# jannerm/ddpo

Measured on AMD Instinct MI355X. Metric: sampled images/sec (512^2, 50 DDIM steps), higher is better.
Workload: dtype f32 (f16mx: f16 MFMA + MX-fp8 cross terms on the long-reduction conv/GEMM layers, bf16x3-split MFMA elsewhere); 1 GPU; BASELINE configs[1]: compressed-animals geometry, sd15 U-Net+VAE (random init), 512x512, 50 DDIM steps, CFG 5.0, eta 1.0, sample_batch_size 8/GPU, VAE decode included; parallelism=dp1, global_batch=8

## Files before the change

### ddpo_amd/csrc/gemm_bf16.hip

```cpp
#include "common.h"
#include <cstdlib>
#include <type_traits>

#ifdef DDPO_KLOOP_TIMING
__device__ unsigned long long ddpo_dbg_t[2 * 16384 * 8];
#define DBG_T(i)                                                                                      \
  do {                                                                                                \
    if (threadIdx.x == 0) {                                                                           \
      const int w_ = (blockIdx.x + gridDim.x * blockIdx.y) & 16383;                                   \
      ddpo_dbg_t[w_ * 8 + (i)] = __builtin_amdgcn_s_memtime();                                        \
      ddpo_dbg_t[w_ * 8 + 4 + (i)] = __builtin_amdgcn_s_memrealtime();                                \
    }                                                                                                 \
  } while (0)
#define DBG_ABL(bit) ((d.splits >> 4) & (bit))
#define DBG_WDECL unsigned long long dbg_w0_ = 0, dbg_wacc_ = 0, dbg_bacc_ = 0
#define DBG_W0() do { dbg_w0_ = __builtin_amdgcn_s_memtime(); } while (0)
#define DBG_WMID() do { const unsigned long long n_ = __builtin_amdgcn_s_memtime(); dbg_wacc_ += n_ - dbg_w0_; dbg_w0_ = n_; } while (0)
#define DBG_W1() do { dbg_bacc_ += __builtin_amdgcn_s_memtime() - dbg_w0_; } while (0)
#define DBG_WSTORE()                                                                 \
  do {                                                                               \
    if (threadIdx.x == 0) {                                                          \
      const int w_ = (blockIdx.x + gridDim.x * blockIdx.y) & 16383;                  \
      ddpo_dbg_t[(16384 + w_) * 8 + 0] = dbg_wacc_;                                  \
      ddpo_dbg_t[(16384 + w_) * 8 + 1] = dbg_bacc_;                                  \
    }                                                                                \
  } while (0)
extern "C" int ddpo_debug_kloop_times(unsigned long long* host, int n_wg) {
  (void)n_wg;
  return hipMemcpyFromSymbol(host, HIP_SYMBOL(ddpo_dbg_t), (size_t)2 * 16384 * 8 * sizeof(unsigned long long)) == hipSuccess ? 0 : -1;
}
#else
#define DBG_T(i) do { } while (0)
#define DBG_ABL(bit) 0
#define DBG_WDECL do { } while (0)
#define DBG_W0() do { } while (0)
#define DBG_WMID() do { } while (0)
#define DBG_W1() do { } while (0)
#define DBG_WSTORE() do { } while (0)
#endif

typedef __bf16 bf16x8 __attribute__((ext_vector_type(8)));
typedef float f32x16 __attribute__((ext_vector_type(16)));
typedef _Float16 f16x8 __attribute__((ext_vector_type(8)));
typedef int i32x8 __attribute__((ext_vector_type(8)));
typedef int i32x4 __attribute__((ext_vector_type(4)));

#define BF_BK 32
#define BF_THREADS 256

__device__ __forceinline__ void split2(float a, float b, uint32_t& hi, uint32_t& lo) {
  hi = cvt_pk_bf16(a, b);
  lo = cvt_pk_bf16(a - __uint_as_float(hi << 16), b - __uint_as_float(hi & 0xFFFF0000u));
}

__device__ __forceinline__ f32x16 mx_mfma(const i32x8 a, const i32x8 b, const f32x16 c, int sa, int opb, int sb) {
  switch (opb) {
    case 0: return __builtin_amdgcn_mfma_scale_f32_32x32x64_f8f6f4(a, b, c, 1, 0, 0, sa, 0, sb);
    case 1: return __builtin_amdgcn_mfma_scale_f32_32x32x64_f8f6f4(a, b, c, 1, 0, 0, sa, 1, sb);
    case 2: return __builtin_amdgcn_mfma_scale_f32_32x32x64_f8f6f4(a, b, c, 1, 0, 0, sa, 2, sb);
    default: return __builtin_amdgcn_mfma_scale_f32_32x32x64_f8f6f4(a, b, c, 1, 0, 0, sa, 3, sb);
  }
}

__device__ __forceinline__ int swz_off(int row, int chunk) { return row * 64 + ((chunk ^ ((row >> 2) & 3)) << 4); }

__device__ __forceinline__ void st_out4(float* p, const float4 v) {
  *reinterpret_cast<float4*>(p) = v;
}

__device__ __forceinline__ void store_planes4(const ddpo_gemm_desc& d, int64_t row, int col, const float4 v) {
  if (d.planes_fmt == 1) {
    mx_store4(d.out_hi, d.out_lo, row, col, d.ld_planes, d.M, v);
    return;
  }
  uint2 h, l;
  split4(v, h, l);
  const int64_t o = plane_off(row, col, d.ld_planes, d.M);
  *reinterpret_cast<uint2*>(d.out_hi + o) = h;
  *reinterpret_cast<uint2*>(d.out_lo + o) = l;
}

constexpr int epi_gcd(int a, int b) { return b == 0 ? a : epi_gcd(b, a % b); }
template <int NIT, int LPR, int WTN, int NBMAX = 10>
struct EpiRows {
  static constexpr int PER = LPR / epi_gcd(64, LPR);
  static constexpr int NB = (NIT % 10 == 0 && NBMAX >= 10) ? 10 : (NIT >= 16 && NIT % 8 == 0 && NBMAX >= 8 ? 8 : (NIT % 5 == 0 && NBMAX >= 5 ? 5 : (NIT % 4 == 0 ? 4 : 1)));
  static constexpr int LB = NIT % 5 == 0 ? 5 : (NIT % 4 == 0 ? 4 : 1);
  float4 bv[PER];
  float4 ex[NB];
  bool any;
  __device__ __forceinline__ void init(const ddpo_gemm_desc& d, int col_base, int lane) {
    any = d.bias || d.rowbias || d.residual || d.alpha != 1.0f;
    if (!any) return;
#pragma unroll
    for (int j = 0; j < PER; ++j) {
      const int e = j * 64 + lane, rr = e / LPR;
      const int colc = min(col_base + (e - rr * LPR) * 4, d.N - 4);
      bv[j] = d.bias ? *reinterpret_cast<const float4*>(d.bias + colc) : make_float4(0.f, 0.f, 0.f, 0.f);
    }
  }
  __device__ __forceinline__ void fetch(const ddpo_gemm_desc& d, int b0, int row_base, int col_base, int lane) {
    if (!d.residual && !d.rowbias) return;
    asm volatile("" : "+v"(lane));
#pragma unroll
    for (int i = 0; i < NB; ++i) {
      const int e = (b0 + i) * 64 + lane, rr = e / LPR;
      const int rowc = min(row_base + rr, d.M - 1), colc = min(col_base + (e - rr * LPR) * 4, d.N - 4);
      ex[i] = d.residual ? *reinterpret_cast<const float4*>(d.residual + (int64_t)rowc * d.ld_res + colc)
                         : *reinterpret_cast<const float4*>(d.rowbias + (int64_t)(rowc / d.rows_per_batch) * d.ld_rowbias + colc);
    }
  }
  __device__ __forceinline__ void combine(const ddpo_gemm_desc& d, float* cw, int b0, int row_base, int col_base, int lane) {
    const bool both = d.residual && d.rowbias;
    asm volatile("" : "+v"(lane));
#pragma unroll
    for (int i = 0; i < NB; ++i) {
      const int it = b0 + i;
      const int e = it * 64 + lane, rr = e / LPR, lcol = (e - rr * LPR) * 4;
      float4 v = *reinterpret_cast<const float4*>(cw + rr * WTN + lcol);
      const float4 b4 = bv[it % PER];
      v.x = d.alpha * v.x + b4.x; v.y = d.alpha * v.y + b4.y; v.z = d.alpha * v.z + b4.z; v.w = d.alpha * v.w + b4.w;
      if (both) {
        const int rowc = min(row_base + rr, d.M - 1), colc = min(col_base + lcol, d.N - 4);
        const float4 rb = *reinterpret_cast<const float4*>(d.rowbias + (int64_t)(rowc / d.rows_per_batch) * d.ld_rowbias + colc);
        v.x += rb.x; v.y += rb.y; v.z += rb.z; v.w += rb.w;
      }
      if (d.residual || d.rowbias) { v.x += ex[i].x; v.y += ex[i].y; v.z += ex[i].z; v.w += ex[i].w; }
      *reinterpret_cast<float4*>(cw + rr * WTN + lcol) = v;
    }
  }
  __device__ __forceinline__ void combine_all(const ddpo_gemm_desc& d, float* cw, int row_base, int col_base, int lane) {
    if (!any) return;
#pragma unroll
    for (int b0 = 0; b0 < NIT; b0 += NB) {
      if (b0) fetch(d, b0, row_base, col_base, lane);
      combine(d, cw, b0, row_base, col_base, lane);
    }
  }
  __device__ __forceinline__ static void emit(const ddpo_gemm_desc& d, const float* cw, int row_base, int col_base, int lane) {
#pragma unroll
    for (int b0 = 0; b0 < NIT; b0 += LB) {
      asm volatile("" : "+v"(lane));
      float4 v[LB];
#pragma unroll
      for (int i = 0; i < LB; ++i) {
        const int e = (b0 + i) * 64 + lane, rr = e / LPR;
        v[i] = *reinterpret_cast<const float4*>(cw + rr * WTN + (e - rr * LPR) * 4);
      }
#pragma unroll
      for (int i = 0; i < LB; ++i) {
        const int e = (b0 + i) * 64 + lane, rr = e / LPR;
        const int row = row_base + rr, col = col_base + (e - rr * LPR) * 4;
        if (row >= d.M || col >= d.N) continue;
        if (d.out) st_out4(d.out + (int64_t)row * d.ld_out + col, v[i]);
        if (d.out_hi) store_planes4(d, row, col, v[i]);
      }
    }
  }
  __device__ __forceinline__ static void partials(const ddpo_gemm_desc& d, const float* cw, float* pp, int row_base, int col_base, int lane) {
#pragma unroll
    for (int it = 0; it < NIT; ++it) {
      const int e = it * 64 + lane, rr = e / LPR, lcol = (e - rr * LPR) * 4;
      const int row = row_base + rr, col = col_base + lcol;
      if (row >= d.M || col >= d.N) continue;
      *reinterpret_cast<float4*>(pp + (int64_t)row * d.N + col) = *reinterpret_cast<const float4*>(cw + rr * WTN + lcol);
    }
  }
};

template <int BM, int BN, int NPASS, bool AFFINE>
__global__ void __launch_bounds__(BF_THREADS) gemm_conv_bf16_kernel(const ddpo_gemm_desc d, const uint16_t* __restrict__ w_hi,
                                                                   const uint16_t* __restrict__ w_lo, int ldw, int tiles_m,
                                                                   int tiles_n, int nblk, int kt_per_split,
                                                                   float* __restrict__ part) {
  constexpr int BK = BF_BK;
  constexpr int TM = BM / 64, TN = BN / 64;
  constexpr int AROWS = BM / 32;
  constexpr int BCH = BN / 64;
  constexpr int NPL = (NPASS == 3) ? 2 : 1;
  constexpr int A_BYTES = BM * 64, B_BYTES = BN * 64;
  extern __shared__ __attribute__((aligned(16))) char smem[];
  constexpr int STAGE = NPL * (A_BYTES + B_BYTES);
  const int t = threadIdx.x, lane = t & 63, wid = t >> 6;
  const int wm = wid >> 1, wn = wid & 1;

  int bid = blockIdx.x;
  {
    const int xcd = bid & 7, idx = bid >> 3;
    const int q = nblk >> 3, r = nblk & 7;
    bid = (xcd < r ? xcd * (q + 1) : r * (q + 1) + (xcd - r) * q) + idx;
  }
  constexpr int GROUP_M = 8;
  const int per_group = GROUP_M * tiles_n;
  const int group = bid / per_group, in_group = bid - group * per_group;
  const int gm0 = group * GROUP_M;
  const int gsz = min(tiles_m - gm0, GROUP_M);
  const int tile_n = in_group / gsz, tile_m = gm0 + (in_group - tile_n * gsz);
  const int m0 = tile_m * BM, n0 = tile_n * BN;

  const bool conv = d.ksize > 0;
  const int VH = d.upsample ? d.H * 2 : d.H, VW = d.upsample ? d.W * 2 : d.W;
  const bool zins = d.upsample == 2;

  const int kq = t & 7;
  const float* arow_ptr[AROWS];
  uint32_t amask[AROWS];
  int aiy0[AROWS], aix0[AROWS];
  int64_t abase[AROWS];
#pragma unroll
  for (int i = 0; i < AROWS; ++i) {
    const int m = m0 + (t >> 3) + 32 * i;
    const bool valid = m < d.M;
    amask[i] = 0;
    if (conv) {
      const int ohw = d.OH * d.OW;
      const int mm = valid ? m : 0;
      const int b = mm / ohw, rem = mm - b * ohw;
      const int oy = rem / d.OW, ox = rem - oy * d.OW;
      const int iy0 = oy * d.stride - d.pad, ix0 = ox * d.stride - d.pad;
      abase[i] = (int64_t)b * d.H * d.W;
      aiy0[i] = iy0; aix0[i] = ix0;
      arow_ptr[i] = d.src + (abase[i] + (int64_t)iy0 * d.W + ix0) * d.ld_src;
      if (AFFINE && valid) {
        for (int ky = 0; ky < d.ksize; ++ky)
          for (int kx = 0; kx < d.ksize; ++kx)
            if (iy0 + ky >= 0 && iy0 + ky < d.H && ix0 + kx >= 0 && ix0 + kx < d.W) amask[i] |= 1u << (ky * d.ksize + kx);
      }
    } else {
      abase[i] = 0; aiy0[i] = aix0[i] = 0;
      arow_ptr[i] = d.src + (int64_t)m * d.ld_src;
      amask[i] = valid ? 1u : 0u;
    }
  }
  const int nk_total = (d.K + BK - 1) / BK;
  const int kt0 = blockIdx.y * kt_per_split;
  const int nk = min(kt_per_split, nk_total - kt0);
// ... 121 lines not shown
      for (int i = 0; i < TM; ++i) {
        ah[i] = *reinterpret_cast<const bf16x8*>(sa + a_ld[ks][i]);
        if (NPASS == 3) al[i] = *reinterpret_cast<const bf16x8*>(sa + A_BYTES + a_ld[ks][i]);
      }
#pragma unroll
      for (int j = 0; j < TN; ++j) {
        bh[j] = *reinterpret_cast<const bf16x8*>(sb + b_ld[ks][j]);
        if (NPASS == 3) bl[j] = *reinterpret_cast<const bf16x8*>(sb + B_BYTES + b_ld[ks][j]);
      }
#pragma unroll
      for (int i = 0; i < TM; ++i)
#pragma unroll
        for (int j = 0; j < TN; ++j) {
          if (NPASS == 3) {
            acc[i][j] = __builtin_amdgcn_mfma_f32_32x32x16_bf16(al[i], bh[j], acc[i][j], 0, 0, 0);
            acc[i][j] = __builtin_amdgcn_mfma_f32_32x32x16_bf16(ah[i], bl[j], acc[i][j], 0, 0, 0);
          }
          acc[i][j] = __builtin_amdgcn_mfma_f32_32x32x16_bf16(ah[i], bh[j], acc[i][j], 0, 0, 0);
        }
    }
  };

  load_tile(0, s0);
  store_tile(0, s0);
  load_tile(1, s0);
  __syncthreads();
  const int nk2 = (nk + 1) & ~1;
#pragma unroll 1
  for (int kt = 0; kt < nk2; kt += 2) {
    load_tile(kt + 2, s1);
    compute(0);
    store_tile(1, s0);
    __syncthreads();
    load_tile(kt + 3, s0);
    compute(1);
    store_tile(0, s1);
    __syncthreads();
  }

  if (part) {
    float* pp = part + (int64_t)blockIdx.y * d.M * d.N;
#pragma unroll
    for (int i = 0; i < TM; ++i)
#pragma unroll
      for (int j = 0; j < TN; ++j) {
        const int col = n0 + wn * (BN / 2) + j * 32 + (lane & 31);
        if (col >= d.N) continue;
#pragma unroll
        for (int r = 0; r < 16; ++r) {
          const int row = m0 + wm * (BM / 2) + i * 32 + (r & 3) + 8 * (r >> 2) + 4 * khalf;
          if (row < d.M) pp[(int64_t)row * d.N + col] = acc[i][j][r];
        }
      }
    return;
  }
#pragma unroll
  for (int i = 0; i < TM; ++i) {
#pragma unroll
    for (int j = 0; j < TN; ++j) {
      const int col = n0 + wn * (BN / 2) + j * 32 + (lane & 31);
      if (col >= d.N) continue;
      const float bv = d.bias ? d.bias[col] : 0.f;
#pragma unroll
      for (int r = 0; r < 16; ++r) {
        const int row = m0 + wm * (BM / 2) + i * 32 + (r & 3) + 8 * (r >> 2) + 4 * khalf;
        if (row >= d.M) continue;
        float v = d.alpha * acc[i][j][r] + bv;
        if (d.rowbias) v += d.rowbias[(int64_t)(row / d.rows_per_batch) * d.ld_rowbias + col];
        if (d.residual) v += d.residual[(int64_t)row * d.ld_res + col];
        d.out[(int64_t)row * d.ld_out + col] = v;
      }
    }
  }
}

typedef unsigned int u32x4 __attribute__((ext_vector_type(4)));
typedef unsigned int u32x2 __attribute__((ext_vector_type(2)));
#define BUF_OOB 0x80000000u

__device__ __forceinline__ __amdgpu_buffer_rsrc_t make_rsrc(const void* p) {
  return __builtin_amdgcn_make_buffer_rsrc(const_cast<void*>(p), 0, 0x7FFFFFFF, 0x00020000);
}

template <int BM, int BN, int NPASS, int ABL = 0, int WM = 2, int WN = 2, bool DEEP = true, int APL = 0>
__global__ void __launch_bounds__(64 * WM * WN, (BM * BN <= 128 * 64 ? 3 : 1)) gemm_conv_bf16_buf_kernel(const ddpo_gemm_desc d, const uint16_t* __restrict__ w_hi,
                                                                       const uint16_t* __restrict__ w_lo, int ldw, int tiles_m,
                                                                       int tiles_n, int nblk, int kt_per_split,
                                                                       float* __restrict__ part) {
  constexpr int BK = BF_BK;
  constexpr int THREADS = 64 * WM * WN;
  constexpr int WTM = BM / WM, WTN = BN / WN;
  constexpr int TM = WTM / 32, TN = WTN / 32;
  constexpr int AR = THREADS / 8, BR = THREADS / 4;
  constexpr int AROWS = BM / AR;
  constexpr int BCH = (BN + BR - 1) / BR;
  constexpr bool BFULL = (BN % BR) == 0;
  static_assert(BM % AR == 0 && WTM % 32 == 0 && WTN % 32 == 0, "tile / wave-grid mismatch");
  constexpr bool MX = NPASS == 4;
  static_assert(!MX || APL == 3 || APL == 7, "the f16mx datapath exists on the plane-fed 128-row tiles (APL 3) and on the tall tile (APL 7)");
  constexpr int NPL = (NPASS == 3 || NPASS == 4) ? 2 : 1;
  constexpr int A_BYTES = BM * 64, B_BYTES = BN * 64;
  extern __shared__ __attribute__((aligned(16))) char smem[];
  constexpr int STAGE = NPL * (A_BYTES + B_BYTES);
  const int t = threadIdx.x, lane = t & 63, wid = t >> 6;
  const int wm = wid / WN, wn = wid % WN;
  DBG_T(0);
  DBG_WDECL;

  int bid = blockIdx.x;
  {
    const int xcd = bid & 7, idx = bid >> 3;
    const int q = nblk >> 3, r = nblk & 7;
    bid = (xcd < r ? xcd * (q + 1) : r * (q + 1) + (xcd - r) * q) + idx;
  }
  constexpr int GROUP_M = 8;
  const int per_group = GROUP_M * tiles_n;
  const int group = bid / per_group, in_group = bid - group * per_group;
  const int gm0 = group * GROUP_M;
  const int gsz = min(tiles_m - gm0, GROUP_M);
  const int tile_n = in_group / gsz, tile_m = gm0 + (in_group - tile_n * gsz);
  const int m0 = tile_m * BM, n0 = tile_n * BN;

  const bool conv = d.ksize > 0;
  const int VH = d.upsample ? d.H * 2 : d.H, VW = d.upsample ? d.W * 2 : d.W;
  const bool zins = d.upsample == 2;
  const int cin = conv ? d.Cin : d.K;
  const int ntaps = conv ? d.ksize * d.ksize : 1;

  f32x16 acc[TM][TN];
#pragma unroll
  for (int i = 0; i < TM; ++i)
#pragma unroll
    for (int j = 0; j < TN; ++j)
#pragma unroll
      for (int r = 0; r < 16; ++r) acc[i][j][r] = 0.f;

  const int khalf = lane >> 5;
  static_assert((WTM % 32) == 0 && (WTN % 32) == 0, "wave sub-tiles are whole 32-row blocks");
  const int a_ld0 = swz_off(wm * WTM + (lane & 31), khalf), b_ld0 = swz_off(wn * WTN + (lane & 31), khalf);
  const int a_ld1 = a_ld0 ^ 32, b_ld1 = b_ld0 ^ 32;

  struct Frag { bf16x8 ah[TM], al[TM], bh[TN], bl[TN]; i32x8 a8[TM], b8[TN]; };
  auto ldfrag_at = [&](const char* sa, const char* sb, int ks, Frag& f) {
    const char* pa = sa + (ks ? a_ld1 : a_ld0);
    const char* pb = sb + (ks ? b_ld1 : b_ld0);
#pragma unroll
    for (int i = 0; i < TM; ++i) {
      f.ah[i] = *reinterpret_cast<const bf16x8*>(pa + i * 2048);
      if (NPASS == 3) f.al[i] = *reinterpret_cast<const bf16x8*>(pa + A_BYTES + i * 2048);
      if (MX && ks) {
        const i32x4 x = *reinterpret_cast<const i32x4*>(sa + a_ld0 + A_BYTES + i * 2048), y = *reinterpret_cast<const i32x4*>(sa + a_ld1 + A_BYTES + i * 2048);
        f.a8[i] = i32x8{x[0], x[1], x[2], x[3], y[0], y[1], y[2], y[3]};
      }
    }
#pragma unroll
    for (int j = 0; j < TN; ++j) {
      f.bh[j] = *reinterpret_cast<const bf16x8*>(pb + j * 2048);
      if (NPASS == 3) f.bl[j] = *reinterpret_cast<const bf16x8*>(pb + B_BYTES + j * 2048);
      if (MX && ks) {
        const i32x4 x = *reinterpret_cast<const i32x4*>(sb + b_ld0 + B_BYTES + j * 2048), y = *reinterpret_cast<const i32x4*>(sb + b_ld1 + B_BYTES + j * 2048);
        f.b8[j] = i32x8{x[0], x[1], x[2], x[3], y[0], y[1], y[2], y[3]};
      }
    }
  };
  auto ldfrag = [&](int cur, int ks, Frag& f) {
    const char* sa = smem + cur * STAGE;
    ldfrag_at(sa, sa + NPL * A_BYTES, ks, f);
  };
  int mx_sa = 0, mx_sbp[(TN + 3) / 4];
  if constexpr (MX) {
    mx_sa = khalf ? 127 - 11 : 127;
#pragma unroll
    for (int q = 0; q < (TN + 3) / 4; ++q) mx_sbp[q] = 0;
#pragma unroll
    for (int j = 0; j < TN; ++j) {
      const int n = n0 + wn * WTN + j * 32 + (lane & 31);
      const int sc = n < d.N ? (int)d.w_scale[n] : 127;
      mx_sbp[j >> 2] |= (khalf ? sc : sc - 11) << (8 * (j & 3));
    }
  }
  auto mma = [&](const Frag& f, int tbeg, int tend, int ks = 0) {
#pragma unroll
    for (int i = 0; i < TM; ++i) {
#pragma unroll
      for (int j = 0; j < TN; ++j) {
        if (i * TN + j < tbeg || i * TN + j >= tend) continue;
        if constexpr (MX) {
          acc[i][j] = __builtin_amdgcn_mfma_f32_32x32x16_f16(__builtin_bit_cast(f16x8, f.ah[i]), __builtin_bit_cast(f16x8, f.bh[j]), acc[i][j], 0, 0, 0);
          if (ks) acc[i][j] = mx_mfma(f.a8[i], f.b8[j], acc[i][j], mx_sa, j & 3, mx_sbp[j >> 2]);
          continue;
        }
        if (NPASS == 3) {
          acc[i][j] = __builtin_amdgcn_mfma_f32_32x32x16_bf16(f.al[i], f.bh[j], acc[i][j], 0, 0, 0);
          acc[i][j] = __builtin_amdgcn_mfma_f32_32x32x16_bf16(f.ah[i], f.bl[j], acc[i][j], 0, 0, 0);
        }
        if constexpr (NPASS == 5) acc[i][j] = __builtin_amdgcn_mfma_f32_32x32x16_f16(__builtin_bit_cast(f16x8, f.ah[i]), __builtin_bit_cast(f16x8, f.bh[j]), acc[i][j], 0, 0, 0);
        else acc[i][j] = __builtin_amdgcn_mfma_f32_32x32x16_bf16(f.ah[i], f.bh[j], acc[i][j], 0, 0, 0);
      }
    }
  };

  if constexpr (APL != 0) {
    static_assert(NPASS == 1 || NPASS == 3 || NPASS == 4 || NPASS == 5, "the plane-fed path: bf16x3 / f16mx (two planes per operand) or single-pass bf16 / f16 (one)");
    constexpr int NW = WM * WN, PAIRS = NPL == 2 ? NW / 2 : NW;
    constexpr int GA = BM / 16, GB = BN / 16;
    static_assert(NW % 2 == 0 && GA % PAIRS == 0 && (NPL == 1 || GB % PAIRS == 0), "pieces must divide evenly over the loader groups");
    constexpr int NA = GA / PAIRS, NB = (GB + PAIRS - 1) / PAIRS;
    constexpr int B_LDS = NB * PAIRS * 1024;
    const int wv = __builtin_amdgcn_readfirstlane(wid);
    const int plane = NPL == 2 ? (wv & 1) : 0, pr = NPL == 2 ? (wv >> 1) : wv;
    const int lr = lane >> 2;
    const uint32_t lc16 = (uint32_t)((lane & 3) ^ ((lane >> 4) & 3)) * 16u;
    const uint64_t a_ptr = reinterpret_cast<uint64_t>(plane ? reinterpret_cast<const void*>(d.w) : reinterpret_cast<const void*>(d.src));
    const uint64_t w_ptr = reinterpret_cast<uint64_t>(plane ? w_lo : w_hi);
    const u32x4 rs_a = {(uint32_t)a_ptr, (uint32_t)(a_ptr >> 32) & 0xFFFFu, 0x7FFFFFFFu, 0x00020000u};
    const u32x4 rs_w = {(uint32_t)w_ptr, (uint32_t)(w_ptr >> 32) & 0xFFFFu, 0x7FFFFFFFu, 0x00020000u};
    const uint32_t lds0 = (uint32_t)(uintptr_t)((__attribute__((address_space(3))) char*)smem);
    const uint32_t lds_a = lds0 + plane * A_BYTES + pr * 1024;
    const uint32_t lds_w = lds0 + NPL * A_BYTES + plane * B_BYTES + pr * 1024;

    const uint32_t a_row_b = d.ld_src == 0 ? 64u : (uint32_t)d.ld_src * 2u;
    const uint32_t a_kt_b = d.ld_src == 0 ? (uint32_t)(conv ? d.B * d.H * d.W : d.M) * 64u : (uint32_t)(BK * 2);
    int aiy0[NA], aix0[NA], apix[NA];
    uint32_t avoff[NA], bvoff[NB];
#pragma unroll
    for (int i = 0; i < NA; ++i) {
      const int m = m0 + 16 * (pr + PAIRS * i) + lr;
      const bool valid = m < d.M;
      if (conv) {
        const int ohw = d.OH * d.OW;
        const int mm = valid ? m : 0;
        const int b = mm / ohw, rem = mm - b * ohw;
        const int oy = rem / d.OW, ox = rem - oy * d.OW;
        aiy0[i] = valid ? oy * d.stride - d.pad : -(1 << 24);
        aix0[i] = ox * d.stride - d.pad;
        apix[i] = b * d.H * d.W;
        avoff[i] = BUF_OOB;
      } else {
        aiy0[i] = aix0[i] = apix[i] = 0;
        avoff[i] = valid ? (uint32_t)m * a_row_b + lc16 : BUF_OOB;
      }
    }
    auto set_tap = [&](int tap) {
      const int ky = d.ksize == 3 ? (tap * 11) >> 5 : 0;
      const int kx = d.ksize == 3 ? tap - ky * 3 : 0;
#pragma unroll
      for (int i = 0; i < NA; ++i) {
        const int iy = aiy0[i] + ky, ix = aix0[i] + kx;
        const bool ok = (unsigned)iy < (unsigned)VH && (unsigned)ix < (unsigned)VW && !(zins && ((iy | ix) & 1));
        const int sy = d.upsample ? (iy >> 1) : iy, sx = d.upsample ? (ix >> 1) : ix;
        const uint32_t off = (uint32_t)(apix[i] + sy * d.W + sx) * a_row_b + lc16;
        avoff[i] = ok ? off : BUF_OOB;
      }
    };
    const uint32_t w_row_b = d.w_layout == 1 ? 64u : (uint32_t)ldw * 2u;
    const uint32_t w_kt_b = d.w_layout == 1 ? (uint32_t)d.N * 64u : (uint32_t)(BK * 2);
#pragma unroll
    for (int i = 0; i < NB; ++i) {
      const int n = n0 + 16 * (pr + PAIRS * i) + lr;
      bool in_tile = true;
      if constexpr (GB % PAIRS != 0) in_tile = pr + PAIRS * i < GB;
      bvoff[i] = (n < d.N && in_tile) ? (uint32_t)n * w_row_b + lc16 : BUF_OOB;
    }
    const int nk_total = d.K / BK;
    const int kt0 = blockIdx.y * kt_per_split;
    const int nk = min(kt_per_split, nk_total - kt0);
    int tap = (kt0 * BK) / cin, cib = kt0 * BK - tap * cin;
    if (conv) set_tap(tap);
    int kt_next = kt0;

    auto fill = [&](int stage) {
      const uint32_t so_a = (uint32_t)(cib >> 5) * a_kt_b, so_w = (uint32_t)kt_next * w_kt_b;
      const uint32_t la = lds_a + stage * STAGE, lw = lds_w + stage * STAGE;
      if (!DBG_ABL(4) || (kt_next - kt0) % 9 < 2) {
#pragma unroll
      for (int i = 0; i < NA; ++i)
        asm volatile("s_nop 4\n\ts_mov_b32 m0, %0\n\ts_nop 0\n\tbuffer_load_dwordx4 %1, %2, %3 offen lds"
                     :: "s"(la + i * (PAIRS * 1024)), "v"(avoff[i]), "s"(rs_a), "s"(so_a) : "memory");
      }
#pragma unroll
      for (int i = 0; i < NB; ++i)
        asm volatile("s_nop 4\n\ts_mov_b32 m0, %0\n\ts_nop 0\n\tbuffer_load_dwordx4 %1, %2, %3 offen lds"
                     :: "s"(lw + i * (PAIRS * 1024)), "v"(bvoff[i]), "s"(rs_w), "s"(so_w) : "memory");
      ++kt_next;
      cib += BK;
      if (cib >= cin) {
        cib = 0; ++tap;
        if (conv && tap < ntaps) set_tap(tap);
      }
    };
    if constexpr (APL == 5 || APL == 6) {
      const bool late = (d.splits & 1) != 0 && wv >= NW / 2;
      auto step4 = [&](int kt, auto cur_c) {
        constexpr int cur = decltype(cur_c)::value;
        DBG_W0();
        asm volatile("s_waitcnt vmcnt(0) lgkmcnt(0)" ::: "memory");
        DBG_WMID();
        __builtin_amdgcn_s_barrier();
        DBG_W1();
        if (kt == 0) DBG_T(1);
        if (kt + 1 < nk && !late && !DBG_ABL(1)) fill(cur ^ 1);
        Frag g;
        ldfrag(cur, 0, g);
        if (!DBG_ABL(2)) mma(g, 0, TM * TN);
        if (kt + 1 < nk && late && !DBG_ABL(1)) fill(cur ^ 1);
        ldfrag(cur, 1, g);
        if (!DBG_ABL(2)) mma(g, 0, TM * TN);
        if (DBG_ABL(2)) asm volatile("" :: "v"(g.ah[0]), "v"(g.bl[TN - 1]), "v"(g.al[TM - 1]), "v"(g.bh[0]));
      };
      {
        const bool rot = wv >= NW / 2;
        fill(0);
        Frag g;
        if (!rot) {
          int kt = 0;
#pragma unroll 1
          for (; kt + 1 < nk; kt += 2) {
            step4(kt, std::integral_constant<int, 0>{});
            step4(kt + 1, std::integral_constant<int, 1>{});
          }
          if (kt < nk) step4(kt, std::integral_constant<int, 0>{});
        } else {
          auto step5 = [&](int kt, auto cur_c) {
            constexpr int cur = decltype(cur_c)::value;
            asm volatile("s_waitcnt vmcnt(0) lgkmcnt(0)" ::: "memory");
            __builtin_amdgcn_s_barrier();
            __builtin_amdgcn_sched_barrier(0);
            if (kt > 0) mma(g, 0, TM * TN);
            __builtin_amdgcn_sched_barrier(0);
            if (kt + 1 < nk) fill(cur ^ 1);
            ldfrag(cur, 0, g);
            mma(g, 0, TM * TN);
            ldfrag(cur, 1, g);
// ... 302 lines not shown
      char* st = smem + buf * STAGE;
#pragma unroll
      for (int i = 0; i < AROWS; ++i) {
        uint2 hi, lo;
        split4(sg.a[i], hi, lo);
        *reinterpret_cast<uint2*>(st + a_st[i]) = hi;
        if (NPASS == 3) *reinterpret_cast<uint2*>(st + A_BYTES + a_st[i]) = lo;
      }
      char* sb = st + NPL * A_BYTES;
#pragma unroll
      for (int i = 0; i < BCH; ++i) {
        if (!BFULL && (t >> 2) + BR * i >= BN) continue;
        *reinterpret_cast<uint4*>(sb + b_st[i]) = sg.bh[i];
        if (NPASS == 3) *reinterpret_cast<uint4*>(sb + B_BYTES + b_st[i]) = sg.bl[i];
      }
    };

    Frag f0, f1;
    constexpr int TT = TM * TN, TH = TT / 2;

    if (ABL & 32) {
#pragma unroll
      for (int i = 0; i < AROWS; ++i) s0.a[i] = make_float4(1.f, 1.f, 1.f, 1.f);
#pragma unroll
      for (int i = 0; i < BCH; ++i) s0.bh[i] = s0.bl[i] = make_uint4(0x3f803f80u, 0x3f803f80u, 0x3f803f80u, 0x3f803f80u);
      store_tile(0, s0);
    } else {
      load_tile(0, s0);
      store_tile(0, s0);
      if (DEEP) load_tile(1, s0);
    }
    __syncthreads();
    DBG_T(1);
    ldfrag(0, 0, f0);
    if (ABL & 8) ldfrag(0, 1, f1);
    if (ABL & 1) s1 = s0;
    const int nk2 = nk & ~1;
#pragma unroll 1
    for (int kt = 0; kt < nk2; kt += 2) {
      if (!(ABL & 1)) { if (DEEP) load_tile(kt + 2, s1); else load_tile(kt + 1, s0); }
      if (!(ABL & 8)) ldfrag(0, 1, f1);
      mma(f0, 0, TT);
      if (!(ABL & 2)) store_tile(1, s0);
      __builtin_amdgcn_sched_barrier(0);
      mma(f1, 0, TH);
      __builtin_amdgcn_sched_barrier(0);
      if (!(ABL & 4)) __syncthreads();
      if (!(ABL & 8)) ldfrag(1, 0, f0);
      __builtin_amdgcn_sched_barrier(0);
      mma(f1, TH, TT);
      if (!(ABL & 1)) { if (DEEP) load_tile(kt + 3, s0); else load_tile(kt + 2, s0); }
      if (!(ABL & 8)) ldfrag(1, 1, f1);
      mma(f0, 0, TT);
      if (!(ABL & 2)) { if (DEEP) store_tile(0, s1); else store_tile(0, s0); }
      __builtin_amdgcn_sched_barrier(0);
      mma(f1, 0, TH);
      __builtin_amdgcn_sched_barrier(0);
      if (!(ABL & 4)) __syncthreads();
      if (!(ABL & 8)) ldfrag(0, 0, f0);
      __builtin_amdgcn_sched_barrier(0);
      mma(f1, TH, TT);
    }
    if (nk & 1) {
      ldfrag(0, 1, f1);
      mma(f0, 0, TT);
      mma(f1, 0, TT);
    }

  }

  DBG_T(2);
  DBG_WSTORE();
  const bool vec_ok = ((d.N | d.ld_out) & 3) == 0 && (reinterpret_cast<uintptr_t>(d.out) & 15) == 0 &&
                      (!d.residual || ((d.ld_res & 3) == 0 && (reinterpret_cast<uintptr_t>(d.residual) & 15) == 0)) &&
                      (!d.rowbias || ((d.ld_rowbias & 3) == 0 && (reinterpret_cast<uintptr_t>(d.rowbias) & 15) == 0)) &&
                      (!d.bias || (reinterpret_cast<uintptr_t>(d.bias) & 15) == 0);
  if constexpr (BM == 256) {
    if (vec_ok) {
      constexpr int LPR = WTN / 4;
      constexpr int NIT = 32 * LPR / 64;
      static_assert((32 * LPR) % 64 == 0, "32-row pass must be a whole number of wave instructions");
      __syncthreads();
      float* cw = reinterpret_cast<float*>(smem) + wid * (32 * WTN);
      float* pp = part ? part + (int64_t)blockIdx.y * d.M * d.N : nullptr;
      using Epi = EpiRows<NIT, LPR, WTN, 5>;
      Epi ep;
      const int colb = n0 + wn * WTN;
      static_assert(TM == 2, "the tall tile's output stage is written for two 32-row passes per wave");
      if constexpr (APL == 6) {
        static_assert(WN == 2 && WTN == 160, "value / gate wave pairs of 160 columns");
        const int oc0 = (n0 / 320) * 160;
        float bj[TN];
#pragma unroll
        for (int j = 0; j < TN; ++j) bj[j] = d.bias ? d.bias[colb + j * 32 + (lane & 31)] : 0.f;
        const float* ca = reinterpret_cast<const float*>(smem) + (wid & ~1) * (32 * WTN);
        const float* cg = ca + 32 * WTN;
        auto gpass = [&](auto IH) {
          constexpr int ih = decltype(IH)::value;
          if (ih > 0) __syncthreads();
#pragma unroll
          for (int j = 0; j < TN; ++j)
#pragma unroll
            for (int r = 0; r < 16; ++r) {
              cw[((r & 3) + 8 * (r >> 2) + 4 * khalf) * WTN + j * 32 + (lane & 31)] = acc[ih][j][r] + bj[j];
            }
          __syncthreads();
          constexpr int GL = WTN / 4;
          int ln = lane;
          asm volatile("" : "+v"(ln));
#pragma unroll
          for (int it = 0; it < 16 * GL / 64; ++it) {
            const int e = it * 64 + ln, rr = wn * 16 + e / GL, c4 = (e - (e / GL) * GL) * 4;
            const float4 a = *reinterpret_cast<const float4*>(ca + rr * WTN + c4);
            const float4 g = *reinterpret_cast<const float4*>(cg + rr * WTN + c4);
            const float4 o = make_float4(a.x * gelu_tanh_f(g.x), a.y * gelu_tanh_f(g.y), a.z * gelu_tanh_f(g.z), a.w * gelu_tanh_f(g.w));
            const int row = m0 + wm * WTM + ih * 32 + rr, col = oc0 + c4;
            if (row >= d.M) continue;
            if (d.aux_out) {
              float* pa = d.aux_out + (int64_t)row * d.N + col;
              *reinterpret_cast<float4*>(pa) = a;
              *reinterpret_cast<float4*>(pa + (d.N >> 1)) = g;
            }
            if (d.out) st_out4(d.out + (int64_t)row * d.ld_out + col, o);
            if (d.out_hi) store_planes4(d, row, col, o);
          }
        };
        gpass(std::integral_constant<int, 0>{});
        gpass(std::integral_constant<int, 1>{});
        DBG_T(3);
        return;
      }
      auto pass = [&](auto IH) {
        constexpr int ih = decltype(IH)::value;
        const int rowb = m0 + wm * WTM + ih * 32;
        if (ih > 0 && !pp) ep.fetch(d, 0, rowb, colb, lane);
#pragma unroll
        for (int j = 0; j < TN; ++j)
#pragma unroll
          for (int r = 0; r < 16; ++r)
            cw[((r & 3) + 8 * (r >> 2) + 4 * khalf) * WTN + j * 32 + (lane & 31)] = acc[ih][j][r];
        if (pp) {
          Epi::partials(d, cw, pp, rowb, colb, lane);
        } else {
          if (ih == 0) { ep.init(d, colb, lane); ep.fetch(d, 0, rowb, colb, lane); }
          ep.combine_all(d, cw, rowb, colb, lane);
          Epi::emit(d, cw, rowb, colb, lane);
        }
      };
      pass(std::integral_constant<int, 0>{});
      pass(std::integral_constant<int, 1>{});
      DBG_T(3);
      return;
    }
  }
  if (vec_ok && !(ABL & 16) && BM != 256) {
    constexpr int LPR = WTN / 4;
    constexpr int NIT = WTM * LPR / 64;
    static_assert((WTM * LPR) % 64 == 0, "wave sub-tile must be a whole number of 1 KiB rows");
    __syncthreads();
    float* cw = reinterpret_cast<float*>(smem) + wid * (WTM * WTN);
    using Epi = EpiRows<NIT, LPR, WTN>;
    Epi ep;
    const int rowb = m0 + wm * WTM, colb = n0 + wn * WTN;
    const bool plain = !part && !(BN == 128 && WN == 2 && WM == 2 && d.epilogue == 1);
    if (plain) { ep.init(d, colb, lane); ep.fetch(d, 0, rowb, colb, lane); }
#pragma unroll
    for (int i = 0; i < TM; ++i)
#pragma unroll
      for (int j = 0; j < TN; ++j)
#pragma unroll
        for (int r = 0; r < 16; ++r)
          cw[(i * 32 + (r & 3) + 8 * (r >> 2) + 4 * khalf) * WTN + j * 32 + (lane & 31)] = acc[i][j][r];
    if (BN == 128 && WN == 2 && WM == 2 && d.epilogue == 1) {
      const int q = (n0 + wn * 64) >> 6;
      const int gc = (lane & 7) * 4, grow = lane >> 3;
      const float4 ba = d.bias ? *reinterpret_cast<const float4*>(d.bias + q * 64 + gc) : make_float4(0.f, 0.f, 0.f, 0.f);
      const float4 bg = d.bias ? *reinterpret_cast<const float4*>(d.bias + q * 64 + 32 + gc) : make_float4(0.f, 0.f, 0.f, 0.f);
#pragma unroll
      for (int it = 0; it < 8; ++it) {
        const int rr = it * 8 + grow;
        const int row = m0 + wm * 64 + rr;
        if (row >= d.M) continue;
        const float4 a = *reinterpret_cast<const float4*>(cw + rr * 64 + gc);
        const float4 g = *reinterpret_cast<const float4*>(cw + rr * 64 + 32 + gc);
        float4 o;
        o.x = (a.x + ba.x) * gelu_tanh_f(g.x + bg.x); o.y = (a.y + ba.y) * gelu_tanh_f(g.y + bg.y);
        o.z = (a.z + ba.z) * gelu_tanh_f(g.z + bg.z); o.w = (a.w + ba.w) * gelu_tanh_f(g.w + bg.w);
        if (d.aux_out) {
          float* pa = d.aux_out + (int64_t)row * d.N + q * 32 + gc;
          *reinterpret_cast<float4*>(pa) = make_float4(a.x + ba.x, a.y + ba.y, a.z + ba.z, a.w + ba.w);
          *reinterpret_cast<float4*>(pa + (d.N >> 1)) = make_float4(g.x + bg.x, g.y + bg.y, g.z + bg.z, g.w + bg.w);
        }
        if (d.out) st_out4(d.out + (int64_t)row * d.ld_out + q * 32 + gc, o);
        if (d.out_hi) store_planes4(d, row, q * 32 + gc, o);
      }
      DBG_T(3);
      return;
    }
    if (part) {
      Epi::partials(d, cw, part + (int64_t)blockIdx.y * d.M * d.N, rowb, colb, lane);
    } else {
      ep.combine_all(d, cw, rowb, colb, lane);
      Epi::emit(d, cw, rowb, colb, lane);
    }
    DBG_T(3);
    return;
  }
  if (part) {
    float* pp = part + (int64_t)blockIdx.y * d.M * d.N;
#pragma unroll
    for (int i = 0; i < TM; ++i)
#pragma unroll
      for (int j = 0; j < TN; ++j) {
        const int col = n0 + wn * WTN + j * 32 + (lane & 31);
        if (col >= d.N) continue;
#pragma unroll
        for (int r = 0; r < 16; ++r) {
          const int row = m0 + wm * WTM + i * 32 + (r & 3) + 8 * (r >> 2) + 4 * khalf;
          if (row < d.M) pp[(int64_t)row * d.N + col] = acc[i][j][r];
        }
      }
    DBG_T(3);
    return;
  }
#pragma unroll
  for (int i = 0; i < TM; ++i) {
#pragma unroll
    for (int j = 0; j < TN; ++j) {
      const int col = n0 + wn * WTN + j * 32 + (lane & 31);
      if (col >= d.N) continue;
      const float bv = d.bias ? d.bias[col] : 0.f;
#pragma unroll
      for (int r = 0; r < 16; ++r) {
        const int row = m0 + wm * WTM + i * 32 + (r & 3) + 8 * (r >> 2) + 4 * khalf;
        if (row >= d.M) continue;
        if ((ABL & 16) && (r | i | j)) { if (acc[i][j][r] == 123.456f) d.out[0] = 1.f; continue; }
        float v = d.alpha * acc[i][j][r] + bv;
        if (d.rowbias) v += d.rowbias[(int64_t)(row / d.rows_per_batch) * d.ld_rowbias + col];
        if (d.residual) v += d.residual[(int64_t)row * d.ld_res + col];
        d.out[(int64_t)row * d.ld_out + col] = v;
      }
    }
  }
  DBG_T(3);
}

__global__ void __launch_bounds__(256) splitk_reduce_kernel(const ddpo_gemm_desc d, const float* __restrict__ part, int splits) {
  const int n4 = d.N >> 2;
  const int64_t total = (int64_t)d.M * n4, mn = (int64_t)d.M * d.N;
  for (int64_t i = (int64_t)blockIdx.x * blockDim.x + threadIdx.x; i < total; i += (int64_t)gridDim.x * blockDim.x) {
    const int row = (int)(i / n4), col = (int)(i - (int64_t)row * n4) << 2;
    float4 a = *reinterpret_cast<const float4*>(part + (int64_t)row * d.N + col);
    for (int s = 1; s < splits; ++s) {
      const float4 b = *reinterpret_cast<const float4*>(part + s * mn + (int64_t)row * d.N + col);
      a.x += b.x; a.y += b.y; a.z += b.z; a.w += b.w;
    }
    float v[4] = {a.x, a.y, a.z, a.w};
#pragma unroll
    for (int e = 0; e < 4; ++e) {
      float x = d.alpha * v[e] + (d.bias ? d.bias[col + e] : 0.f);
      if (d.rowbias) x += d.rowbias[(int64_t)(row / d.rows_per_batch) * d.ld_rowbias + col + e];
      if (d.residual) x += d.residual[(int64_t)row * d.ld_res + col + e];
      v[e] = x;
      if (d.out) d.out[(int64_t)row * d.ld_out + col + e] = x;
    }
    if (d.out_hi) store_planes4(d, row, col, make_float4(v[0], v[1], v[2], v[3]));
  }
}

static bool planes_out_ok(const ddpo_gemm_desc& d) {
  if (!d.out_hi) return d.out != nullptr && !d.out_lo;
  if (!d.out_lo || d.ld_planes < 0 || (d.ld_planes & 3)) return false;
  if ((reinterpret_cast<uintptr_t>(d.out_hi) | reinterpret_cast<uintptr_t>(d.out_lo)) & 7) return false;
  const int ncols = d.epilogue != 0 ? d.N / 2 : d.N;
  if (d.ld_planes == 0 ? (ncols & 31) != 0 : d.ld_planes < ncols) return false;
  if (d.planes_fmt != 0 && (d.planes_fmt != 1 || (ncols & 31) || (d.ld_planes & 31))) return false;
  if (d.N & 3) return false;
  if (d.out && ((d.ld_out & 3) || (reinterpret_cast<uintptr_t>(d.out) & 15))) return false;
  if (d.residual && ((d.ld_res & 3) || (reinterpret_cast<uintptr_t>(d.residual) & 15))) return false;
  if (d.rowbias && ((d.ld_rowbias & 3) || (reinterpret_cast<uintptr_t>(d.rowbias) & 15))) return false;
  if (d.bias && (reinterpret_cast<uintptr_t>(d.bias) & 15)) return false;
  return true;
}

enum { TC_TALL = 0, TC_WIDE = 1, TC_128 = 2, TC_64 = 3, TC_GENERIC = 4, TC_SPLITK_REDUCE = 5, TC_MX = 6, TC_COUNT = 8 };
static unsigned long long g_tile_launches[TC_COUNT] = {0, 0, 0, 0, 0, 0, 0, 0};
extern "C" int ddpo_gemm_tile_launch_counts(unsigned long long* out_host, int n) {
  if (!out_host || n < TC_COUNT) return DDPO_EINVAL;
  for (int i = 0; i < TC_COUNT; ++i) out_host[i] = __atomic_load_n(&g_tile_launches[i], __ATOMIC_RELAXED);
  return DDPO_OK;
}
static inline void count_tile(int cls) { __atomic_fetch_add(&g_tile_launches[cls], 1ull, __ATOMIC_RELAXED); }

static bool g_force_generic = false;
static bool buf_path_ok(const ddpo_gemm_desc& d, int ldw) {
  if (g_force_generic) return false;
  const int64_t lim = 0x7FFFFFFF;
  if (d.w_layout == 1) ldw = (d.K + 31) / 32 * 32;
  if (d.ksize > 0) {
    if (d.Cin % BF_BK) return false;
    if ((int64_t)d.B * d.H * d.W * (d.ld_src ? d.ld_src : d.Cin) * 4 >= lim) return false;
    const int64_t wbytes = d.w_dgrad ? (int64_t)d.K * d.N * 2 : (int64_t)d.N * ldw * 2;
    if (wbytes >= lim) return false;
  } else {
    if (d.K % BF_BK) return false;
    if ((int64_t)d.M * (d.ld_src ? d.ld_src : d.K) * 4 >= lim || (int64_t)d.N * ldw * 2 >= lim) return false;
  }
  return true;
}
#ifdef DDPO_DEBUG_HOOKS
extern "C" void ddpo_debug_force_generic_gemm(int on) { g_force_generic = on != 0; }
#endif

template <int BM, int BN, int NPASS, int WM = 2, int WN = 2, int APL = 0>
static int launch_bf16(const ddpo_gemm_desc& d, const uint16_t* w_hi, const uint16_t* w_lo, int ldw, float* ws, size_t ws_bytes,
                       hipStream_t st) {
  const int tiles_m = (d.M + BM - 1) / BM, tiles_n = (d.N + BN - 1) / BN;
  const int nblk = tiles_m * tiles_n;
  const int nk_total = (d.K + BF_BK - 1) / BF_BK;
  int splits = 1;
  if (ws && nblk < 192 && nk_total >= 32 && (d.N & 3) == 0 && d.epilogue == 0) {
    splits = (384 + nblk - 1) / nblk;
    if (splits > 8) splits = 8;
    if (splits > nk_total / 8) splits = nk_total / 8;
    while (splits > 1 && (size_t)splits * d.M * d.N * sizeof(float) > ws_bytes) --splits;
  }
  int ktps = (nk_total + splits - 1) / splits;
  ktps = (ktps + 1) & ~1;
  splits = (nk_total + ktps - 1) / ktps;
  float* part = splits > 1 ? ws : nullptr;
  constexpr int NPL = (NPASS == 3 || NPASS == 4) ? 2 : 1;
  size_t lds = (APL == 3) ? NPL * (size_t)(2 * BM + 3 * BN) * 64 : 2 * NPL * (size_t)(BM + BN) * 64;
  if (lds < (size_t)BM * BN * 4) lds = (size_t)BM * BN * 4;
  static bool attr_set = false;
  if (!attr_set) {
    if constexpr (APL == 0) {
      (void)hipFuncSetAttribute(reinterpret_cast<const void*>(&gemm_conv_bf16_kernel<BM, BN, NPASS, true>),
                                hipFuncAttributeMaxDynamicSharedMemorySize, (int)lds);
      (void)hipFuncSetAttribute(reinterpret_cast<const void*>(&gemm_conv_bf16_kernel<BM, BN, NPASS, false>),
                                hipFuncAttributeMaxDynamicSharedMemorySize, (int)lds);
    }
    (void)hipFuncSetAttribute(reinterpret_cast<const void*>(&gemm_conv_bf16_buf_kernel<BM, BN, NPASS, 0, WM, WN, true, APL>),
                              hipFuncAttributeMaxDynamicSharedMemorySize, (int)lds);
    attr_set = true;
  }
  count_tile(BN == 128 ? TC_128 : TC_64);
  if constexpr (NPASS == 4) count_tile(TC_MX);
  if constexpr (APL != 0) {
    hipLaunchKernelGGL((gemm_conv_bf16_buf_kernel<BM, BN, NPASS, 0, WM, WN, true, APL>), dim3(nblk, splits), dim3(64 * WM * WN), lds, st, d, w_hi,
                       w_lo, ldw, tiles_m, tiles_n, nblk, ktps, part);
  } else {
    if (!buf_path_ok(d, ldw)) count_tile(TC_GENERIC);
    if (buf_path_ok(d, ldw))
      hipLaunchKernelGGL((gemm_conv_bf16_buf_kernel<BM, BN, NPASS, 0, WM, WN, true, APL>), dim3(nblk, splits), dim3(64 * WM * WN), lds, st, d, w_hi,
                         w_lo, ldw, tiles_m, tiles_n, nblk, ktps, part);
    else if (d.upsample == 0)
      hipLaunchKernelGGL((gemm_conv_bf16_kernel<BM, BN, NPASS, true>), dim3(nblk, splits), dim3(BF_THREADS), lds, st, d, w_hi, w_lo, ldw,
                         tiles_m, tiles_n, nblk, ktps, part);
    else
      hipLaunchKernelGGL((gemm_conv_bf16_kernel<BM, BN, NPASS, false>), dim3(nblk, splits), dim3(BF_THREADS), lds, st, d, w_hi, w_lo, ldw,
                         tiles_m, tiles_n, nblk, ktps, part);
  }
  DDPO_LAUNCH_CHECK();
  if (splits > 1) {
    int64_t blocks = ((int64_t)d.M * (d.N >> 2) + 255) / 256;
    if (blocks > 4096) blocks = 4096;
    count_tile(TC_SPLITK_REDUCE);
    hipLaunchKernelGGL(splitk_reduce_kernel, dim3((int)blocks), dim3(256), 0, st, d, part, splits);
    DDPO_LAUNCH_CHECK();
  }
  return DDPO_OK;
}


static int wide_splits(const ddpo_gemm_desc& d, bool have_ws, size_t ws_bytes) {
  const int nblk = ((d.M + 127) / 128) * ((d.N + 319) / 320);
  const int nk_total = d.K / BF_BK;
  int splits = 1;
  if (have_ws && nblk <= 192 && nk_total >= 16) {
    splits = (256 + nblk / 2) / nblk;
    if (splits > 8) splits = 8;
    if (splits > nk_total / 8) splits = nk_total / 8;
    if (splits < 1) splits = 1;
    while (splits > 1 && (size_t)splits * d.M * d.N * sizeof(float) > ws_bytes) --splits;
  }
  return splits;
}

template <int NPASS, int APL = 0>
static int launch_bf16_wide(const ddpo_gemm_desc& d, const uint16_t* w_hi, const uint16_t* w_lo, int ldw, float* ws, size_t ws_bytes,
                            hipStream_t st) {
  constexpr int BM = 128, BN = 320, WM = 4, WN = 2;
  const int tiles_m = (d.M + BM - 1) / BM, tiles_n = (d.N + BN - 1) / BN;
  const int nblk = tiles_m * tiles_n;
  const int nk_total = d.K / BF_BK;
  int splits = wide_splits(d, ws != nullptr, ws_bytes);
  int ktps = (nk_total + splits - 1) / splits;
  ktps = (ktps + 1) & ~1;
  splits = (nk_total + ktps - 1) / ktps;
  float* part = splits > 1 ? ws : nullptr;
  const size_t lds = (size_t)BM * BN * 4;
  static bool attr_set = false;
  if (!attr_set) {
    (void)hipFuncSetAttribute(reinterpret_cast<const void*>(&gemm_conv_bf16_buf_kernel<BM, BN, NPASS, 0, WM, WN, true, APL>),
                              hipFuncAttributeMaxDynamicSharedMemorySize, (int)lds);
    attr_set = true;
  }
  count_tile(TC_WIDE);
  if constexpr (NPASS == 4) count_tile(TC_MX);
  hipLaunchKernelGGL((gemm_conv_bf16_buf_kernel<BM, BN, NPASS, 0, WM, WN, true, APL>), dim3(nblk, splits), dim3(64 * WM * WN), lds, st, d, w_hi,
                     w_lo, ldw, tiles_m, tiles_n, nblk, ktps, part);
  DDPO_LAUNCH_CHECK();
  if (splits > 1) {
    int64_t blocks = ((int64_t)d.M * (d.N >> 2) + 255) / 256;
    if (blocks > 4096) blocks = 4096;
    count_tile(TC_SPLITK_REDUCE);
    hipLaunchKernelGGL(splitk_reduce_kernel, dim3((int)blocks), dim3(256), 0, st, d, part, splits);
    DDPO_LAUNCH_CHECK();
  }
  return DDPO_OK;
}

template <int APL, int NPASS = 3>
static int launch_bf16_tall(const ddpo_gemm_desc& d, const uint16_t* w_hi, const uint16_t* w_lo, int ldw, hipStream_t st) {
  constexpr int BM = 256, BN = 320, WM = 4, WN = 2;
  const int tiles_m = (d.M + BM - 1) / BM, tiles_n = (d.N + BN - 1) / BN;
  const int nblk = tiles_m * tiles_n;
  const int nk_total = d.K / BF_BK;
  const size_t lds = 8 * 32 * 160 * 4;
  static bool attr_set = false;
  if (!attr_set) {
    (void)hipFuncSetAttribute(reinterpret_cast<const void*>(&gemm_conv_bf16_buf_kernel<BM, BN, NPASS, 0, WM, WN, true, APL>),
                              hipFuncAttributeMaxDynamicSharedMemorySize, (int)lds);
    attr_set = true;
  }
  count_tile(TC_TALL);
  hipLaunchKernelGGL((gemm_conv_bf16_buf_kernel<BM, BN, NPASS, 0, WM, WN, true, APL>), dim3(nblk, 1), dim3(64 * WM * WN), lds, st, d, w_hi, w_lo, ldw,
                     tiles_m, tiles_n, nblk, nk_total, (float*)nullptr);
  DDPO_LAUNCH_CHECK();
  return DDPO_OK;
}

static int launch_mx_tall(const ddpo_gemm_desc& d, const uint16_t* w16, const uint16_t* w8, hipStream_t st) {
  constexpr int BM = 256, BN = 320, WM = 4, WN = 2;
  const int tiles_m = (d.M + BM - 1) / BM, tiles_n = (d.N + BN - 1) / BN;
  const int nblk = tiles_m * tiles_n;
  const int nk_total = d.K / BF_BK;
  const size_t lds = 8 * 32 * 160 * 4;
  static bool attr_set = false;
  if (!attr_set) {
    (void)hipFuncSetAttribute(reinterpret_cast<const void*>(&gemm_conv_bf16_buf_kernel<BM, BN, 4, 0, WM, WN, true, 7>),
                              hipFuncAttributeMaxDynamicSharedMemorySize, (int)lds);
    attr_set = true;
  }
  count_tile(TC_TALL);
  count_tile(TC_MX);
  hipLaunchKernelGGL((gemm_conv_bf16_buf_kernel<BM, BN, 4, 0, WM, WN, true, 7>), dim3(nblk, 1), dim3(64 * WM * WN), lds, st, d, w16, w8, 0,
                     tiles_m, tiles_n, nblk, nk_total, (float*)nullptr);
  DDPO_LAUNCH_CHECK();
  return DDPO_OK;
}

template <int APL>
static int dispatch_bf16(const ddpo_gemm_desc& d, const uint16_t* w_hi, const uint16_t* w_lo, int ldw, int npass, void* ws, size_t ws_bytes,
                         hipStream_t st) {
  if (d.epilogue != 0) {
    if ((d.epilogue != 1 && d.epilogue != 2) || (d.N & 127) || !buf_path_ok(d, ldw) || d.rowbias || d.residual || d.alpha != 1.0f || d.w_dgrad) return DDPO_EINVAL;
    if ((d.ld_out & 3) || (reinterpret_cast<uintptr_t>(d.out) & 15) || (d.bias && (reinterpret_cast<uintptr_t>(d.bias) & 15))) return DDPO_EINVAL;
    if (reinterpret_cast<uintptr_t>(d.aux_out) & 15) return DDPO_EINVAL;
    if (d.epilogue == 2) {
      if constexpr (APL == 3) {
        if (npass != 3 || d.N % 320 || ((d.N >> 1) & 3)) return DDPO_EINVAL;
        return launch_bf16_tall<6>(d, w_hi, w_lo, ldw, st);
      }
      return DDPO_EINVAL;
    }
    if constexpr (APL == 3) {
      if (npass == 4) return launch_bf16<128, 128, 4, 2, 2, 3>(d, w_hi, w_lo, ldw, nullptr, 0, st);
      if (npass == 1) return launch_bf16<128, 128, 1, 2, 2, 3>(d, w_hi, w_lo, ldw, nullptr, 0, st);
      if (npass == 5) return launch_bf16<128, 128, 5, 2, 2, 3>(d, w_hi, w_lo, ldw, nullptr, 0, st);
    }
    return npass == 3 ? launch_bf16<128, 128, 3, 2, 2, APL>(d, w_hi, w_lo, ldw, nullptr, 0, st) : launch_bf16<128, 128, 1>(d, w_hi, w_lo, ldw, nullptr, 0, st);
  }
  float* wsf = (ws && !(reinterpret_cast<uintptr_t>(ws) & 15)) ? reinterpret_cast<float*>(ws) : nullptr;
  constexpr int wide_mode = 1;
  if constexpr (APL != 0) {
    constexpr int tall_mode = 1;
    const long ntall = (long)((d.M + 255) / 256) * (d.N / 320), nwide = (long)((d.M + 127) / 128) * (d.N / 320);
    const double eff_tall = (double)ntall / (double)(((ntall + 255) / 256) * 256), eff_wide = (double)nwide / (double)(((nwide + 255) / 256) * 256);
    if (tall_mode && npass == 3 && d.N % 320 == 0 && d.epilogue == 0 && ntall >= 200 && eff_tall * 1.08 >= eff_wide)
      return launch_bf16_tall<5>(d, w_hi, w_lo, ldw, st);
    if constexpr (APL == 3) {
      if (npass == 1 && d.N % 320 == 0 && d.epilogue == 0 && ntall >= 200 && eff_tall * 1.08 >= eff_wide)
        return launch_bf16_tall<8, 1>(d, w_hi, w_lo, ldw, st);
      if (npass == 5 && d.N % 320 == 0 && d.epilogue == 0 && ntall >= 200 && eff_tall * 1.08 >= eff_wide)
        return launch_bf16_tall<8, 5>(d, w_hi, w_lo, ldw, st);
      const char* mx_tall_env = getenv("DDPO_MX_TALL");
      if (npass == 4 && !(mx_tall_env && mx_tall_env[0] == '0') && d.N % 320 == 0 && d.epilogue == 0 && ntall >= 200 && eff_tall * 1.08 >= eff_wide)
        return launch_mx_tall(d, w_hi, w_lo, st);
    }
  }
  const int wsplits = wide_splits(d, wsf != nullptr, ws_bytes);
  if (wide_mode && d.N % 320 == 0 && d.M >= 512 && buf_path_ok(d, ldw) && !(d.K / BF_BK < 16 && d.N > 1280) &&
      (long)((d.M + 127) / 128) * (d.N / 320) * wsplits >= 200 &&
      !(wsplits > 1 && d.K / BF_BK < 64)) {
    if constexpr (APL == 3) {
      if (npass == 4) return launch_bf16_wide<4, 3>(d, w_hi, w_lo, ldw, wsf, ws_bytes, st);
      if (npass == 1) return launch_bf16_wide<1, 3>(d, w_hi, w_lo, ldw, wsf, ws_bytes, st);
      if (npass == 5) return launch_bf16_wide<5, 3>(d, w_hi, w_lo, ldw, wsf, ws_bytes, st);
    }
    return npass == 3 ? launch_bf16_wide<3, APL>(d, w_hi, w_lo, ldw, wsf, ws_bytes, st) : launch_bf16_wide<1>(d, w_hi, w_lo, ldw, wsf, ws_bytes, st);
  }
  const long t128 = (long)((d.M + 127) / 128) * ((d.N + 127) / 128);
  constexpr long big_min = 256;
  constexpr int mid64 = 1;
  const bool mid_short = mid64 && t128 < 512 && d.K / BF_BK <= 64;
  const bool big = (d.N % 128 == 0) && t128 >= big_min && !mid_short;
  if constexpr (APL == 3) {
    if (npass == 4)
      return big ? launch_bf16<128, 128, 4, 2, 2, 3>(d, w_hi, w_lo, ldw, wsf, ws_bytes, st) : launch_bf16<128, 64, 4, 2, 2, 3>(d, w_hi, w_lo, ldw, wsf, ws_bytes, st);
    if (npass == 1)
      return big ? launch_bf16<128, 128, 1, 2, 2, 3>(d, w_hi, w_lo, ldw, wsf, ws_bytes, st) : launch_bf16<128, 64, 1, 2, 2, 3>(d, w_hi, w_lo, ldw, wsf, ws_bytes, st);
    if (npass == 5)
      return big ? launch_bf16<128, 128, 5, 2, 2, 3>(d, w_hi, w_lo, ldw, wsf, ws_bytes, st) : launch_bf16<128, 64, 5, 2, 2, 3>(d, w_hi, w_lo, ldw, wsf, ws_bytes, st);
  }
  if (npass == 3)
    return big ? launch_bf16<128, 128, 3, 2, 2, APL>(d, w_hi, w_lo, ldw, wsf, ws_bytes, st) : launch_bf16<128, 64, 3, 2, 2, APL>(d, w_hi, w_lo, ldw, wsf, ws_bytes, st);
  return big ? launch_bf16<128, 128, 1>(d, w_hi, w_lo, ldw, wsf, ws_bytes, st) : launch_bf16<128, 64, 1>(d, w_hi, w_lo, ldw, wsf, ws_bytes, st);
}

extern "C" int ddpo_gemm_conv_fwd_bf16(const ddpo_gemm_desc* dp, const uint16_t* w_hi, const uint16_t* w_lo, int ldw, int npass,
                                       void* ws, size_t ws_bytes, void* stream) {
  if (!dp || !w_hi) return DDPO_EINVAL;
  const ddpo_gemm_desc& d = *dp;
  if (npass != 1 && npass != 3) return DDPO_EINVAL;
  if (npass == 3 && !w_lo) return DDPO_EINVAL;
  if (!d.src || d.M <= 0 || d.N <= 0 || d.K <= 0 || d.ld_src <= 0 || (d.ld_src & 3) || (reinterpret_cast<uintptr_t>(d.src) & 15)) return DDPO_EINVAL;
  if ((reinterpret_cast<uintptr_t>(w_hi) & 15) || (w_lo && (reinterpret_cast<uintptr_t>(w_lo) & 15))) return DDPO_EINVAL;
  if (!planes_out_ok(d) || (d.out_hi && !buf_path_ok(d, ldw))) return DDPO_EINVAL;
  if (d.ksize > 0) {
    if (d.ksize != 1 && d.ksize != 3) return DDPO_EINVAL;
    if ((d.Cin & 7) || d.K != d.ksize * d.ksize * d.Cin || d.M != d.B * d.OH * d.OW) return DDPO_EINVAL;
    if (d.upsample < 0 || d.upsample > 2) return DDPO_EINVAL;
  } else if (d.K & 7) {
    return DDPO_EINVAL;
  }
  if (d.w_layout != 0 && (d.w_layout != 1 || d.w_dgrad)) return DDPO_EINVAL;
  if (d.w_dgrad) {
    if (d.ksize <= 0 || (d.Cin & 7)) return DDPO_EINVAL;
  } else if (d.w_layout == 0 && (ldw < d.K || (ldw & 7))) {
    return DDPO_EINVAL;
  }
  return dispatch_bf16<0>(d, w_hi, w_lo, ldw, npass, ws, ws_bytes, as_stream(stream));
}

extern "C" int ddpo_gemm_conv_fwd_bf16_planes(const ddpo_gemm_desc* dp, const uint16_t* a_hi, const uint16_t* a_lo, int lda,
                                              const uint16_t* w_hi, const uint16_t* w_lo, int ldw, void* ws, size_t ws_bytes,
                                              void* stream) {
  if (!dp || !a_hi || !w_hi || (a_lo == nullptr) != (w_lo == nullptr)) return DDPO_EINVAL;
  const int npass = a_lo ? 3 : 1;
  ddpo_gemm_desc d = *dp;
  if (d.M <= 0 || d.N <= 0 || d.K <= 0 || lda < 0 || (lda & 7) || d.w_dgrad || !planes_out_ok(d)) return DDPO_EINVAL;
  if (npass == 1 && d.epilogue == 2) return DDPO_EINVAL;
  if ((reinterpret_cast<uintptr_t>(a_hi) | reinterpret_cast<uintptr_t>(a_lo) | reinterpret_cast<uintptr_t>(w_hi) |
       reinterpret_cast<uintptr_t>(w_lo)) & 15) return DDPO_EINVAL;
  if (d.w_layout != 0 && d.w_layout != 1) return DDPO_EINVAL;
  if (d.w_layout == 0 && (ldw < d.K || (ldw & 7))) return DDPO_EINVAL;
  if (d.ksize > 0) {
    if (d.ksize != 1 && d.ksize != 3) return DDPO_EINVAL;
    if (d.K != d.ksize * d.ksize * d.Cin || d.M != d.B * d.OH * d.OW || d.upsample < 0 || d.upsample > 2 || (lda && lda < d.Cin)) return DDPO_EINVAL;
  } else if (lda && lda < d.K) {
    return DDPO_EINVAL;
  }
  d.src = reinterpret_cast<const float*>(a_hi);
  d.w = reinterpret_cast<const float*>(a_lo);
  d.ld_src = lda;
  if (!buf_path_ok(d, ldw)) return DDPO_EINVAL;
  d.splits = 1;
#ifdef DDPO_KLOOP_TIMING
  { const char* e = getenv("DDPO_DBG_ABL"); if (e) d.splits |= atoi(e) << 4; }
#endif
  return dispatch_bf16<3>(d, w_hi, w_lo, ldw, npass, ws, ws_bytes, as_stream(stream));
}

extern "C" int ddpo_gemm_conv_fwd_f16mx_planes(const ddpo_gemm_desc* dp, const uint16_t* a16, const uint16_t* a8, int lda,
                                               const uint16_t* w16, const uint16_t* w8, void* ws, size_t ws_bytes, void* stream) {
  if (!dp || !a16 || !w16 || (a8 == nullptr) != (w8 == nullptr) || (a8 && !dp->w_scale)) return DDPO_EINVAL;
  const int npass = a8 ? 4 : 5;
  ddpo_gemm_desc d = *dp;
  if (npass == 5 && d.epilogue == 2) return DDPO_EINVAL;
  if (d.M <= 0 || d.N <= 0 || d.K <= 0 || lda < 0 || (lda & 31) || d.w_dgrad || d.w_layout != 1 || !planes_out_ok(d)) return DDPO_EINVAL;
  if ((reinterpret_cast<uintptr_t>(a16) | reinterpret_cast<uintptr_t>(a8) | reinterpret_cast<uintptr_t>(w16) | reinterpret_cast<uintptr_t>(w8)) & 15)
    return DDPO_EINVAL;
  if (d.ksize > 0) {
    if (d.ksize != 1 && d.ksize != 3) return DDPO_EINVAL;
    if (d.K != d.ksize * d.ksize * d.Cin || d.M != d.B * d.OH * d.OW || d.upsample < 0 || d.upsample > 2 || (lda && lda < d.Cin)) return DDPO_EINVAL;
  } else if (lda && lda < d.K) {
    return DDPO_EINVAL;
  }
  d.src = reinterpret_cast<const float*>(a16);
  d.w = reinterpret_cast<const float*>(a8);
  d.ld_src = lda;
  if (!buf_path_ok(d, 0)) return DDPO_EINVAL;
  d.splits = 1;
#ifdef DDPO_KLOOP_TIMING
  { const char* e = getenv("DDPO_DBG_ABL"); if (e) d.splits |= atoi(e) << 4; }
#endif
  return dispatch_bf16<3>(d, w16, w8, 0, npass, ws, ws_bytes, as_stream(stream));
}

__global__ void __launch_bounds__(256) pack_weights_kernel(const float* __restrict__ w, int K, int N, int Kp,
                                                           uint16_t* __restrict__ fwd_hi, uint16_t* __restrict__ fwd_lo,
                                                           uint16_t* __restrict__ bwd_hi, uint16_t* __restrict__ bwd_lo) {
  __shared__ uint32_t tile[32][33];
  const int k0 = blockIdx.y * 32, n0 = blockIdx.x * 32;
  const int tx = threadIdx.x & 31, ty = threadIdx.x >> 5;
  for (int r = ty; r < 32; r += 8) {
    const int k = k0 + r, n = n0 + tx;
    uint32_t packed = 0;
    if (k < K && n < N) {
      const float x = w[(int64_t)k * N + n];
      const uint32_t h = cvt_pk_bf16(x, 0.f) & 0xFFFFu;
      const float rem = x - __uint_as_float(h << 16);
      const uint32_t l = cvt_pk_bf16(rem, 0.f) & 0xFFFFu;
      packed = h | (l << 16);
      if (bwd_hi) { bwd_hi[(int64_t)k * N + n] = (uint16_t)h; bwd_lo[(int64_t)k * N + n] = (uint16_t)l; }
    }
    tile[r][tx] = packed;
  }
  __syncthreads();
  for (int r = ty; r < 32; r += 8) {
    const int n = n0 + r, k = k0 + tx;
    if (n < N && k < Kp) {
      const uint32_t p = tile[tx][r];
      fwd_hi[(int64_t)n * Kp + k] = (uint16_t)(p & 0xFFFFu);
      fwd_lo[(int64_t)n * Kp + k] = (uint16_t)(p >> 16);
    }
  }
}

__global__ void __launch_bounds__(256) pack_weights_kblocked_kernel(const float* __restrict__ w, int K, int N, uint16_t* __restrict__ fwd_hi,
                                                                    uint16_t* __restrict__ fwd_lo) {
  __shared__ uint32_t tile[32][33];
  const int kb = blockIdx.y, k0 = kb * 32, n0 = blockIdx.x * 32;
  const int tx = threadIdx.x & 31, ty = threadIdx.x >> 5;
  for (int r = ty; r < 32; r += 8) {
    const int k = k0 + r, n = n0 + tx;
    uint32_t packed = 0;
    if (k < K && n < N) {
      const float x = w[(int64_t)k * N + n];
      const uint32_t h = cvt_pk_bf16(x, 0.f) & 0xFFFFu;
      const float rem = x - __uint_as_float(h << 16);
      packed = h | ((cvt_pk_bf16(rem, 0.f) & 0xFFFFu) << 16);
    }
    tile[r][tx] = packed;
  }
  __syncthreads();
  for (int r = ty; r < 32; r += 8) {
    const int n = n0 + r;
    if (n < N) {
      const uint32_t p = tile[tx][r];
      const int64_t o = ((int64_t)kb * N + n) * 32 + tx;
      fwd_hi[o] = (uint16_t)(p & 0xFFFFu);
      fwd_lo[o] = (uint16_t)(p >> 16);
    }
  }
}

extern "C" int ddpo_pack_weights_bf16_kblocked(const float* w, int K, int N, uint16_t* fwd_hi, uint16_t* fwd_lo, void* stream) {
  if (!w || !fwd_hi || !fwd_lo || K <= 0 || N <= 0) return DDPO_EINVAL;
  dim3 grid((N + 31) / 32, (K + 31) / 32);
  hipLaunchKernelGGL(pack_weights_kblocked_kernel, grid, dim3(256), 0, as_stream(stream), w, K, N, fwd_hi, fwd_lo);
  DDPO_LAUNCH_CHECK();
  return DDPO_OK;
}

__global__ void __launch_bounds__(256) pack_weights_kblocked_dgrad_kernel(const float* __restrict__ w, int taps, int Cin, int Cout,
                                                                          uint16_t* __restrict__ hi, uint16_t* __restrict__ lo) {
  const int kb = blockIdx.y, tx = threadIdx.x & 31, ty = threadIdx.x >> 5;
  const int Kd = taps * Cout;
  const int k = kb * 32 + tx;
  const bool kok = k < Kd;
  const int tap = kok ? k / Cout : 0, co = k - tap * Cout;
  const float* src = w + ((int64_t)(taps - 1 - tap) * Cin) * Cout + co;
  for (int r = ty; r < 32; r += 8) {
    const int n = blockIdx.x * 32 + r;
    if (n >= Cin) continue;
    uint32_t h = 0, l = 0;
    if (kok) {
      const float x = src[(int64_t)n * Cout];
      h = cvt_pk_bf16(x, 0.f) & 0xFFFFu;
// ... 731 lines not shown
```

### ddpo_amd/lib.py

```python
import ctypes
import os
import threading
from ctypes import c_void_p, c_int, c_int32, c_int64, c_uint32, c_float, c_double, c_size_t, POINTER, byref

import torch

_HERE = os.path.dirname(os.path.abspath(__file__))
LIB_PATH = os.path.join(_HERE, "libddpo_hip.so")

PRED_TYPES = {"epsilon": 0, "v_prediction": 1, "sample": 2}


class LoraLayer(ctypes.Structure):
    _fields_ = [("w0", c_void_p), ("w", c_void_p), ("a", c_void_p), ("b", c_void_p), ("K", c_int), ("N", c_int), ("r", c_int), ("s", c_float)]


class DdimConsts(ctypes.Structure):
    _fields_ = [("alphas_cumprod", c_void_p), ("num_train_timesteps", c_int), ("step_ratio", c_int),
                ("final_alpha_cumprod", c_float), ("eta", c_float), ("pred_type", c_int)]


class GemmDesc(ctypes.Structure):
    _fields_ = [("src", c_void_p), ("ld_src", c_int),
                ("w", c_void_p), ("w_trans", c_int),
                ("bias", c_void_p),
                ("rowbias", c_void_p), ("rows_per_batch", c_int), ("ld_rowbias", c_int),
                ("residual", c_void_p), ("ld_res", c_int),
                ("out", c_void_p), ("ld_out", c_int),
                ("alpha", c_float),
                ("M", c_int), ("N", c_int), ("K", c_int),
                ("ksize", c_int), ("stride", c_int), ("pad", c_int), ("upsample", c_int),
                ("B", c_int), ("H", c_int), ("W", c_int), ("Cin", c_int),
                ("OH", c_int), ("OW", c_int),
                ("w_dgrad", c_int), ("ld_w", c_int), ("splits", c_int), ("accumulate", c_int), ("epilogue", c_int),
                ("out_hi", c_void_p), ("out_lo", c_void_p), ("ld_planes", c_int), ("w_layout", c_int),
                ("w_scale", c_void_p), ("planes_fmt", c_int), ("colsum", c_void_p), ("aux_out", c_void_p)]


ABI_VERSION = 14

_SIGS = {
    "ddpo_abi_version": (c_int, []),
    "ddpo_sizeof_gemm_desc": (c_size_t, []),
    "ddpo_sizeof_ddim_consts": (c_size_t, []),
    "ddpo_gemm_tile_launch_counts": (c_int, [c_void_p, c_int]),
    "ddpo_threefry_bits_host": (c_int, [c_uint32, c_uint32, c_int64, c_void_p]),
    "ddpo_threefry_normal": (c_int, [c_uint32, c_uint32, c_void_p, c_void_p, c_int64, c_void_p]),
    "ddpo_ddim_step_fwd": (c_int, [c_void_p, c_void_p, c_void_p, c_void_p, c_void_p, c_float, POINTER(DdimConsts),
                                   c_void_p, c_void_p, c_int, c_int, c_void_p]),
    "ddpo_ddim_logprob_ppo_fwd_bwd": (c_int, [c_void_p, c_void_p, c_void_p, c_void_p, c_void_p, c_void_p, c_void_p,
                                              c_float, c_float, c_int, POINTER(DdimConsts), c_void_p, c_void_p,
                                              c_void_p, c_void_p, c_int, c_int, c_void_p]),
    "ddpo_ddim_logprob_ppo_fwd_bwd_grouped": (c_int, [c_void_p, c_void_p, c_void_p, c_void_p, c_void_p, c_void_p, c_void_p,
                                                      c_float, c_float, c_int, POINTER(DdimConsts), c_void_p, c_void_p,
                                                      c_void_p, c_void_p, c_int, c_int, c_int, c_void_p]),
    "ddpo_rwr_noisy_latents": (c_int, [c_void_p, c_void_p, c_void_p, c_void_p, c_void_p, c_int, c_float, c_void_p, c_void_p, c_int, c_int, c_int,
                                       c_void_p]),
    "ddpo_rwr_mse_fwd_bwd": (c_int, [c_void_p, c_void_p, c_void_p, c_void_p, c_float, c_int, c_void_p, c_void_p, c_void_p, c_void_p, c_int, c_int,
                                     c_void_p]),
    "ddpo_grad_sqnorm": (c_int, [c_void_p, c_int64, c_void_p, c_int, c_void_p]),
    "ddpo_adamw_bf16mu_step": (c_int, [c_void_p, c_void_p, c_void_p, c_void_p, c_int64, c_void_p, c_double, c_double,
                                       c_double, c_double, c_double, c_double, c_double, c_int, c_int, c_int, c_void_p]),
    "ddpo_groupnorm_ws_bytes": (c_size_t, [c_int, c_int, c_int, c_int]),
    "ddpo_groupnorm_fwd": (c_int, [c_void_p, c_int, c_void_p, c_int, c_void_p, c_void_p, c_int, c_int, c_int, c_int,
                                   c_float, c_int, c_void_p, c_void_p, c_void_p]),
    "ddpo_layernorm_fwd": (c_int, [c_void_p, c_void_p, c_void_p, c_void_p, c_int, c_int, c_float, c_void_p]),
    "ddpo_gemm_conv_fwd": (c_int, [POINTER(GemmDesc), c_void_p]),
    "ddpo_gemm_conv_wgrad": (c_int, [POINTER(GemmDesc), c_void_p]),
    "ddpo_gemm_conv_fwd_bf16": (c_int, [POINTER(GemmDesc), c_void_p, c_void_p, c_int, c_int, c_void_p, c_size_t, c_void_p]),
    "ddpo_gemm_conv_wgrad_bf16x3": (c_int, [POINTER(GemmDesc), c_void_p]),
    "ddpo_gemm_conv_wgrad_bf16x3_planes": (c_int, [POINTER(GemmDesc), c_void_p, c_void_p, c_void_p, c_void_p, c_void_p]),
    "ddpo_gemm_conv_fwd_bf16_planes": (c_int, [POINTER(GemmDesc), c_void_p, c_void_p, c_int, c_void_p, c_void_p, c_int, c_void_p, c_size_t,
                                               c_void_p]),
    "ddpo_split_planes_bf16": (c_int, [c_void_p, c_int, c_void_p, c_void_p, c_int, c_int64, c_int, c_void_p]),
    "ddpo_groupnorm_fwd_planes": (c_int, [c_void_p, c_int, c_void_p, c_void_p, c_int, c_void_p, c_void_p, c_int, c_int, c_int, c_int,
                                          c_float, c_int, c_void_p, c_void_p, c_void_p]),
    "ddpo_layernorm_fwd_planes": (c_int, [c_void_p, c_void_p, c_void_p, c_void_p, c_void_p, c_int, c_int, c_float, c_int, c_void_p]),
    "ddpo_pack_weights_bf16": (c_int, [c_void_p, c_int, c_int, c_int, c_void_p, c_void_p, c_void_p, c_void_p, c_void_p]),
    "ddpo_pack_weights_bf16_kblocked": (c_int, [c_void_p, c_int, c_int, c_void_p, c_void_p, c_void_p]),
    "ddpo_pack_weights_bf16_kblocked_dgrad": (c_int, [c_void_p, c_int, c_int, c_int, c_void_p, c_void_p, c_void_p]),
    "ddpo_pack_weights_f16mx": (c_int, [c_void_p, c_int, c_int, c_void_p, c_void_p, c_void_p, c_void_p]),
    "ddpo_split_planes_f16mx": (c_int, [c_void_p, c_int, c_void_p, c_void_p, c_int, c_int64, c_int, c_void_p]),
    "ddpo_gemm_conv_fwd_f16mx_planes": (c_int, [POINTER(GemmDesc), c_void_p, c_void_p, c_int, c_void_p, c_void_p, c_void_p, c_size_t, c_void_p]),
    "ddpo_attention_fwd": (c_int, [c_void_p, c_int, c_void_p, c_int, c_void_p, c_int, c_void_p, c_int, c_void_p, c_int, c_int,
                                   c_int, c_int, c_int, c_float, c_void_p]),
    "ddpo_attention_kv_images_bytes": (c_size_t, [c_int, c_int, c_int, c_int]),
    "ddpo_attention_pack_kv_bf16x3": (c_int, [c_void_p, c_int, c_void_p, c_int, c_void_p, c_size_t, c_int, c_int, c_int, c_int, c_void_p]),
    "ddpo_attention_fwd_bf16x3_images": (c_int, [c_void_p, c_int, c_void_p, c_size_t, c_void_p, c_int, c_void_p, c_int, c_int, c_int, c_int, c_int,
                                                 c_float, c_void_p]),
    "ddpo_attention_fwd_bf16x3": (c_int, [c_void_p, c_int, c_void_p, c_int, c_void_p, c_int, c_void_p, c_int, c_void_p, c_int, c_int,
                                          c_int, c_int, c_int, c_float, c_void_p, c_size_t, c_void_p]),
    "ddpo_attention_fwd_bf16x3_ws_bytes": (c_size_t, [c_int, c_int, c_int, c_int]),
    "ddpo_attention_fwd_f16p": (c_int, [c_void_p, c_int, c_void_p, c_int, c_void_p, c_int, c_void_p, c_int, c_void_p, c_int, c_int,
                                        c_int, c_int, c_int, c_float, c_void_p, c_size_t, c_void_p]),
    "ddpo_attention_pack_kv_f16p": (c_int, [c_void_p, c_int, c_void_p, c_int, c_void_p, c_size_t, c_int, c_int, c_int, c_int, c_void_p]),
    "ddpo_attention_fwd_f16p_images": (c_int, [c_void_p, c_int, c_void_p, c_size_t, c_void_p, c_int, c_void_p, c_int, c_int, c_int, c_int, c_int,
                                               c_float, c_void_p]),
    **{f"ddpo_attention_fwd_{v}_po": (c_int, [c_void_p, c_int, c_void_p, c_int, c_void_p, c_int, c_void_p, c_void_p, c_int, c_void_p, c_int, c_int,
                                              c_int, c_int, c_int, c_float, c_void_p, c_size_t, c_void_p]) for v in ("bf16x3", "f16p")},
    **{f"ddpo_attention_fwd_{v}_images_po": (c_int, [c_void_p, c_int, c_void_p, c_size_t, c_void_p, c_void_p, c_int, c_void_p, c_int, c_int, c_int,
                                                     c_int, c_int, c_float, c_void_p]) for v in ("bf16x3", "f16p")},
    "ddpo_attention_bwd_f16p": (c_int, [c_void_p, c_int, c_void_p, c_int, c_void_p, c_int, c_void_p, c_void_p, c_void_p, c_void_p,
                                        c_void_p, c_void_p, c_void_p, c_int, c_int, c_int, c_int, c_int, c_float, c_void_p]),
    "ddpo_attention_bwd": (c_int, [c_void_p, c_int, c_void_p, c_int, c_void_p, c_int, c_void_p, c_void_p, c_void_p, c_void_p,
                                   c_void_p, c_void_p, c_void_p, c_int, c_int, c_int, c_int, c_int, c_float, c_void_p]),
    "ddpo_attention_bwd_bf16x3": (c_int, [c_void_p, c_int, c_void_p, c_int, c_void_p, c_int, c_void_p, c_void_p, c_void_p, c_void_p,
                                          c_void_p, c_void_p, c_void_p, c_int, c_int, c_int, c_int, c_int, c_float, c_void_p]),
    "ddpo_groupnorm_stats_floats": (c_size_t, [c_int, c_int, c_int]),
    "ddpo_groupnorm_bwd_ws_bytes": (c_size_t, [c_int, c_int, c_int, c_int]),
    "ddpo_groupnorm_bwd": (c_int, [c_void_p, c_int, c_void_p, c_int, c_void_p, c_void_p, c_int, c_int, c_int, c_int, c_int,
                                   c_void_p, c_int, c_void_p, c_int, c_void_p, c_void_p, c_void_p, c_void_p]),
    "ddpo_layernorm_bwd": (c_int, [c_void_p, c_void_p, c_void_p, c_int, c_int, c_float, c_void_p, c_void_p, c_void_p, c_void_p, c_void_p, c_void_p]),
    "ddpo_layernorm_bwd_ws_bytes": (c_size_t, [c_int, c_int]),
    "ddpo_geglu_bwd": (c_int, [c_void_p, c_void_p, c_void_p, c_int64, c_int, c_void_p]),
    "ddpo_silu_bwd": (c_int, [c_void_p, c_void_p, c_void_p, c_int64, c_void_p]),
    "ddpo_colsum_accum": (c_int, [c_void_p, c_int, c_int64, c_int, c_int, c_void_p, c_void_p]),
    "ddpo_sumpool2x2": (c_int, [c_void_p, c_void_p, c_int, c_int, c_int, c_int, c_void_p]),
    "ddpo_add": (c_int, [c_void_p, c_void_p, c_void_p, c_int64, c_void_p]),
    "ddpo_geglu_fwd": (c_int, [c_void_p, c_void_p, c_int64, c_int, c_void_p]),
    "ddpo_silu_fwd": (c_int, [c_void_p, c_void_p, c_int64, c_void_p]),
    "ddpo_quick_gelu_fwd": (c_int, [c_void_p, c_void_p, c_int64, c_void_p]),
    "ddpo_l2_normalize_rows": (c_int, [c_void_p, c_void_p, c_int, c_int, c_void_p]),
    "ddpo_timestep_embedding": (c_int, [c_void_p, c_void_p, c_int, c_int, c_void_p]),
    "ddpo_nchw_to_nhwc": (c_int, [c_void_p, c_void_p, c_int, c_int, c_int, c_void_p]),
    "ddpo_nhwc_to_nchw": (c_int, [c_void_p, c_void_p, c_int, c_int, c_int, c_void_p]),
    "ddpo_copy_cols": (c_int, [c_void_p, c_int, c_void_p, c_int, c_int64, c_int, c_void_p]),
    "ddpo_stage_cfg_inputs": (c_int, [c_void_p, c_void_p, c_int64, c_void_p, c_void_p, c_int, c_void_p, c_void_p, c_int, c_void_p]),
    "ddpo_softmax_rows": (c_int, [c_void_p, c_int64, c_int, c_float, c_void_p]),
    "ddpo_scale_shift_clip": (c_int, [c_void_p, c_void_p, c_int64, c_float, c_float, c_float, c_float, c_void_p]),
    "ddpo_lora_merge": (c_int, [c_void_p, c_int, c_int64, c_void_p]),
    "ddpo_lora_wgrad_ws_bytes": (c_size_t, [c_int, c_int, c_int, c_int]),
    "ddpo_lora_wgrad": (c_int, [c_void_p, c_int, c_void_p, c_void_p, c_int, c_void_p, c_int, c_void_p, c_void_p, c_void_p, c_void_p,
                                c_int, c_int, c_int, c_int, c_float, c_void_p, c_size_t, c_void_p]),
    "ddpo_attention_causal_fwd": (c_int, [c_void_p, c_int, c_void_p, c_int, c_void_p, c_int, c_void_p, c_int, c_int, c_int, c_int, c_int, c_float, c_void_p]),
    "ddpo_gather_rows": (c_int, [c_void_p, c_int, c_int, c_void_p, c_int, c_int, c_void_p, c_int, c_void_p, c_void_p]),
    "ddpo_cosine_rows": (c_int, [c_void_p, c_void_p, c_int, c_int, c_float, c_void_p, c_void_p]),
}

EXPORTED_SYMBOLS = tuple(_SIGS)
_lib = None
DATAPATH = os.environ.get("DDPO_DATAPATH", "fp32")


DATAPATHS = ("fp32", "bf16x3", "bf16", "f16mx")
SHIPPED_DATAPATH = "f16mx"


def shipped_datapath():
    name = os.environ.get("DDPO_DATAPATH") or SHIPPED_DATAPATH
    if name not in DATAPATHS:
        raise ValueError(f"DDPO_DATAPATH={name!r}: expected one of {DATAPATHS}")
    return name


MX_CROSS = os.environ.get("DDPO_MX_CROSS", "1") == "1"
MX_MIN_K = int(os.environ.get("DDPO_MX_MIN_K", "2560"))
_TLS = threading.local()


def current_datapath():
    return getattr(_TLS, "datapath", None) or DATAPATH


class datapath:

    def __init__(self, name):
# ... 371 lines not shown
                                         int(step_t), int(mu_decay_in_bf16), int(zero_grad), _stream()), "ddpo_adamw_bf16mu_step")


_ws_cache = {}


def _scratch(nbytes, device, tag):
    key = (tag, str(device), torch.cuda.current_stream().cuda_stream)
    ws = _ws_cache.get(key)
    if ws is None or ws.numel() < nbytes:
        ws = torch.empty(max(int(nbytes), 1 << 20), dtype=torch.uint8, device=device)
        _ws_cache[key] = ws
    return ws


def groupnorm(x, B, HW, gamma, beta, groups, eps, silu, out=None, ld_x=None, ld_out=None, return_stats=False, planes=False):
    C = gamma.numel()
    if ld_x is None and x.dim() == 2 and x.stride(0) != C:
        ld_x = x.stride(0)
    _p = _p_rows if ld_x else globals()["_p"]
    if planes:
        pl = Planes(B * HW, C, x.device, fmt=1 if planes == 2 else 0)
        ws = _scratch(load().ddpo_groupnorm_ws_bytes(B, HW, C, groups), x.device, "gn")
        stats = torch.empty(load().ddpo_groupnorm_stats_floats(B, C, groups), dtype=torch.float32, device=x.device)
        _p2 = globals()["_p"]
        _check(load().ddpo_groupnorm_fwd_planes(_p(x), int(ld_x or C), _p2(pl.hi), _p2(pl.lo), pl.ld, _p2(gamma), _p2(beta), B, HW, C, groups,
                                                float(eps), int(bool(silu)) | (2 * pl.fmt), _p2(ws), _p2(stats), _stream()), "ddpo_groupnorm_fwd_planes")
        return (pl, stats) if return_stats else pl
    if out is None:
        out = torch.empty(B * HW, C, dtype=torch.float32, device=x.device)
    ws = _scratch(load().ddpo_groupnorm_ws_bytes(B, HW, C, groups), x.device, "gn")
    stats = torch.empty(load().ddpo_groupnorm_stats_floats(B, C, groups), dtype=torch.float32, device=x.device)
    _p2 = globals()["_p"]
    _check(load().ddpo_groupnorm_fwd(_p(x), int(ld_x or C), _p2(out), int(ld_out or C), _p2(gamma), _p2(beta), B, HW, C, groups,
                                     float(eps), int(bool(silu)), _p2(ws), _p2(stats), _stream()), "ddpo_groupnorm_fwd")
    return (out, stats) if return_stats else out


def groupnorm_bwd(x, dy, stats, gamma, B, HW, groups, silu, dgamma, dbeta, dx_add=None, ld_x=None, ld_dy=None):
    C = gamma.numel()
    dx = torch.empty(B * HW, C, dtype=torch.float32, device=x.device)
    ws = _scratch(load().ddpo_groupnorm_bwd_ws_bytes(B, HW, C, groups), x.device, "gnb")
    _check(load().ddpo_groupnorm_bwd(_p(x), int(ld_x or C), _p(dy), int(ld_dy or C), _p(stats), _p(gamma), B, HW, C, groups,
                                     int(bool(silu)), _p(dx_add), C, _p(dx), C, _p(dgamma), _p(dbeta), _p(ws), _stream()),
           "ddpo_groupnorm_bwd")
    return dx


def layernorm(x, gamma, beta, eps=1e-5, out=None, planes=False):
    rows, C = x.shape
    if planes:
        pl = Planes(rows, C, x.device, fmt=1 if planes == 2 else 0)
        _check(load().ddpo_layernorm_fwd_planes(_p(x), _p(pl.hi), _p(pl.lo), _p(gamma), _p(beta), rows, C, float(eps), int(pl.kblocked) | (2 * pl.fmt), _stream()),
               "ddpo_layernorm_fwd_planes")
        return pl
    if out is None:
        out = torch.empty_like(x)
    _check(load().ddpo_layernorm_fwd(_p(x), _p(out), _p(gamma), _p(beta), rows, C, float(eps), _stream()), "ddpo_layernorm_fwd")
    return out


def pack_weights(w, bwd=True):
    N = w.shape[-1]
    K = w.numel() // N
    Kp = (K + 7) // 8 * 8
    ent = PACKED.get(w.data_ptr())
    mk = lambda *s: torch.zeros(*s, dtype=torch.int16, device=w.device)
    lay = 1 if (W_KBLOCKED and N % 4 == 0) else 0
    if lay:
        Kp = (K + 31) // 32 * 32
    if ent is None or ent["K"] != K or ent["N"] != N or ent.get("w_layout", 0) != lay:
        ent = dict(K=K, N=N, fwd=(mk(N, Kp), mk(N, Kp), Kp), bwd=None, w_layout=lay)
        PACKED[w.data_ptr()] = ent
    n_dg = w.shape[2] if w.dim() == 4 else K
    dg_ok = bool(bwd and DGRAD_FWD and _x3() and W_KBLOCKED and w.dim() in (2, 4) and N % 32 == 0 and n_dg % 4 == 0)
    if dg_ok:
        _pack_dgrad_planes(w, ent)
    else:
        ent.pop("dg", None)
    if bwd and ent["bwd"] is None and not dg_ok:
        ent["bwd"] = (mk(K, N), mk(K, N))
    if "geglu" in ent:
        ent["geglu"]["stale"] = True
    fh, fl, _ = ent["fwd"]
    bh, bl = ent["bwd"] if ent["bwd"] is not None else (None, None)
    if _mx() and K % 32 == 0 and K >= MX_MIN_K:
        if "mx" not in ent:
            ent["mx"] = dict(w16=torch.zeros(K // 32, N, 32, dtype=torch.int16, device=w.device), w8=torch.zeros(K // 32, N, 64, dtype=torch.uint8, device=w.device),
                             scale=torch.zeros(N, dtype=torch.uint8, device=w.device))
        m = ent["mx"]
        _check(load().ddpo_pack_weights_f16mx(_p(w), K, N, _p(m["w16"]), _p(m["w8"]), _p(m["scale"]), _stream()), "ddpo_pack_weights_f16mx")
    else:
        ent.pop("mx", None)
    if ent["w_layout"] == 1:
        _check(load().ddpo_pack_weights_bf16_kblocked(_p(w), K, N, _p(fh), _p(fl), _stream()), "ddpo_pack_weights_bf16_kblocked")
        if bh is not None:
            _check(load().ddpo_split_planes_bf16(_p(w), N, _p(bh), _p(bl), N, K, N, _stream()), "ddpo_split_planes_bf16")
    else:
        _check(load().ddpo_pack_weights_bf16(_p(w), K, N, Kp, _p(fh), _p(fl), _p(bh), _p(bl), _stream()), "ddpo_pack_weights_bf16")
    return ent


def _pack_dgrad_planes(w, ent):
    taps = w.shape[0] * w.shape[1] if w.dim() == 4 else 1
    Nd, cout = (w.shape[2], w.shape[3]) if w.dim() == 4 else (w.shape[0], w.shape[1])
    Kd = taps * cout
    Kp = (Kd + 31) // 32 * 32
    dg = ent.get("dg")
    if dg is None or dg["K"] != Kd or dg["N"] != Nd:
        mk = lambda *sh: torch.zeros(*sh, dtype=torch.int16, device=w.device)
        dg = ent["dg"] = dict(K=Kd, N=Nd, hi=mk(Nd, Kp), lo=mk(Nd, Kp))
    _check(load().ddpo_pack_weights_bf16_kblocked_dgrad(_p(w), taps, Nd, cout, _p(dg["hi"]), _p(dg["lo"]), _stream()), "ddpo_pack_weights_bf16_kblocked_dgrad")
    return dg


def _dgrad_fwd(dy, dg, *, M, conv=None, residual=None, ld_res=None, out=None):
    Kd, Nd = dg["K"], dg["N"]
    cin = conv["Cin"] if conv else Kd
    rows = conv["B"] * conv["H"] * conv["W"] if conv else M
    lim = 0x7FFFFFFF
    if conv is None and rows * cin * 4 >= lim and not isinstance(dy, Planes):
        step = (lim - 1) // (cin * 4) // 256 * 256
        if step <= 0:
            raise DdpoHipError(f"_dgrad_fwd: one 256-row chunk of a {cin}-wide dY does not fit the buffer-addressed kernels")
        if out is None:
            out = torch.empty(M, Nd, dtype=torch.float32, device=dy.device)
        for r0 in range(0, rows, step):
            r1 = min(rows, r0 + step)
            assert (r1 - r0) * cin * 4 < lim
            _dgrad_fwd(dy[r0:r1], dg, M=r1 - r0, residual=None if residual is None else residual[r0:r1], ld_res=ld_res, out=out[r0:r1])
        return out
    buf_ok = cin % 32 == 0 and rows * cin * 4 < lim and Nd * ((Kd + 31) // 32 * 32) * 2 < lim
    pl = dy if isinstance(dy, Planes) else None
    if pl is not None and (pl.fmt != 0 or not buf_ok):
        dy, pl = pl.float(), None
    if pl is None and buf_ok and PLANES and (Kd >= 2560 or PLANES_ALL):
        pl = split_planes(dy)
    d = GemmDesc()
    dev = pl.device if pl is not None else dy.device
    if out is None:
        out = torch.empty(M, Nd, dtype=torch.float32, device=dev)
    if residual is not None:
        d.residual = residual.data_ptr(); d.ld_res = int(ld_res if ld_res is not None else Nd)
    d.out = out.data_ptr(); d.ld_out = int(Nd)
    d.alpha = 1.0
    d.M, d.N, d.K = int(M), int(Nd), int(Kd)
    d.w_layout = 1
    if conv:
        for k in ("ksize", "stride", "pad", "upsample", "B", "H", "W", "Cin", "OH", "OW"):
            setattr(d, k, int(conv[k]))
    ws = _scratch(SPLITK_WS_BYTES, dev, "splitk")
    if pl is not None:
        _check(load().ddpo_gemm_conv_fwd_bf16_planes(byref(d), _p(pl.hi), _p(pl.lo), pl.ld, _p(dg["hi"]), _p(dg["lo"]), 0, _p(ws), SPLITK_WS_BYTES, _stream()),
               "ddpo_gemm_conv_fwd_bf16_planes(dgrad)")
    else:
        d.src = dy.data_ptr(); d.ld_src = int(cin)
        _check(load().ddpo_gemm_conv_fwd_bf16(byref(d), _p(dg["hi"]), _p(dg["lo"]), 0, 3, _p(ws), SPLITK_WS_BYTES, _stream()), "ddpo_gemm_conv_fwd_bf16(dgrad)")
    return out


def pack_weights_geglu(w, bias):
    K, N = w.shape
    F = N // 2
    if current_datapath() == "fp32" or (N % 128) or (K % 32):
        return False
    ent = PACKED.get(w.data_ptr())
    if ent is None:
        return False
    mk = lambda: torch.zeros(N, K, dtype=torch.int16, device=w.device)
    if "geglu" not in ent:
        idx = torch.arange(F, device=w.device).view(F // 32, 1, 32)
        perm = torch.cat([idx, idx + F], dim=1).reshape(-1)
        ent["geglu"] = dict(perm=perm, hi=mk(), lo=mk(), bias=torch.empty(N, dtype=torch.float32, device=w.device), w_layout=1 if W_KBLOCKED else 0)
    g = ent["geglu"]
    wp = w.index_select(1, g["perm"]).contiguous()
    torch.index_select(bias, 0, g["perm"], out=g["bias"])
    if g["w_layout"] == 1:
        _check(load().ddpo_pack_weights_bf16_kblocked(_p(wp), K, N, _p(g["hi"]), _p(g["lo"]), _stream()), "ddpo_pack_weights_bf16_kblocked")
    else:
        _check(load().ddpo_pack_weights_bf16(_p(wp), K, N, K, _p(g["hi"]), _p(g["lo"]), None, None, _stream()), "ddpo_pack_weights_bf16")
    if GEGLU_TALL and W_KBLOCKED and _x3() and N % 320 == 0 and not (_mx() and K >= MX_MIN_K):
        if "tall" not in g:
            idx = torch.arange(F, device=w.device).view(F // 160, 1, 160)
# ... 655 lines not shown
```

### ddpo_amd/models/unet.py

```python
import math
import re
from collections import OrderedDict
from dataclasses import dataclass
from typing import Tuple

import os

import torch

from .. import lib as L


@dataclass(frozen=True)
class UNetConfig:
    in_channels: int = 4
    out_channels: int = 4
    block_out_channels: Tuple[int, ...] = (320, 640, 1280, 1280)
    cross_attn_down: Tuple[bool, ...] = (True, True, True, False)
    layers_per_block: int = 2
    num_heads: Tuple[int, ...] = (8, 8, 8, 8)
    cross_attention_dim: int = 768
    use_linear_projection: bool = False
    norm_groups: int = 32
    prediction_type: str = "epsilon"

    @staticmethod
    def named(name):
        if name in ("sd15", "sd14", "sd1"):
            return UNetConfig()
        if name == "sd21":
            return UNetConfig(num_heads=(5, 10, 20, 20), cross_attention_dim=1024, use_linear_projection=True,
                              prediction_type="v_prediction")
        if name == "tiny":
            return UNetConfig(block_out_channels=(32, 64, 128, 128), cross_attention_dim=64)
        if name == "tiny21":
            return UNetConfig(block_out_channels=(32, 64, 128, 128), num_heads=(2, 4, 8, 8), cross_attention_dim=96,
                              use_linear_projection=True, prediction_type="v_prediction")
        raise KeyError(name)


class ParamStore:

    def __init__(self, shapes, device):
        self.shapes = OrderedDict(shapes)
        self.offsets = OrderedDict()
        off = 0
        for name, shp in self.shapes.items():
            self.offsets[name] = off
            off += (math.prod(shp) + 3) // 4 * 4
        self.numel = off
        self.n_params = sum(math.prod(s) for s in self.shapes.values())
        self.flat = torch.zeros(off, dtype=torch.float32, device=device)
        self.views = {n: self.flat[o:o + math.prod(self.shapes[n])].view(self.shapes[n]) for n, o in self.offsets.items()}
        self.fused_qkv = {}

    def __getitem__(self, name):
        return self.views[name]

    def __contains__(self, name):
        return name in self.views

    def load_dict(self, tree):
        missing = [n for n in self.shapes if n not in tree]
        if missing:
            raise KeyError(f"missing parameters: {missing[:5]}{'...' if len(missing) > 5 else ''}")
        for n, v in self.views.items():
            t = torch.as_tensor(tree[n], dtype=torch.float32)
            if tuple(t.shape) != tuple(self.shapes[n]):
                raise ValueError(f"{n}: expected {self.shapes[n]}, got {tuple(t.shape)}")
            v.copy_(t)

    def pack_bf16(self, bwd=True, names=None):
        if names is not None:
            sel = set(names)
            qkv = []
            for n, v in self.views.items():
                if n not in sel or not n.endswith(".kernel"):
                    continue
                L.pack_weights(v, bwd=bwd)
                if n.endswith(".ff.net_0.proj.kernel"):
                    L.pack_weights_geglu(v, self.views[n[:-len("kernel")] + "bias"])
                m = re.search(r"\.attn1\.to_[qkv]\.kernel$", n)
                if QKV_FUSED and m and n[:m.start()] + ".attn1." not in qkv:
                    qkv.append(n[:m.start()] + ".attn1.")
            for pre in qkv:
                self._pack_fused_qkv(pre)
            return
        for n, v in self.views.items():
            if n.endswith(".kernel"):
                L.pack_weights(v, bwd=bwd)
                if n.endswith(".ff.net_0.proj.kernel"):
                    L.pack_weights_geglu(v, self.views[n[:-len("kernel")] + "bias"])
                if QKV_FUSED and n.endswith(".attn1.to_q.kernel"):
                    self._pack_fused_qkv(n[:-len("to_q.kernel")])

    def _pack_fused_qkv(self, pre):
        v = self.views[pre + "to_q.kernel"]
        parts = [v, self.views[pre + "to_k.kernel"], self.views[pre + "to_v.kernel"]]
        buf = self.fused_qkv.get(pre)
        if buf is None:
            buf = self.fused_qkv[pre] = torch.empty(v.shape[0], sum(t.shape[1] for t in parts), dtype=torch.float32, device=v.device)
        torch.cat(parts, dim=1, out=buf)
        L.pack_weights(buf, bwd=False)

    def init_synthetic(self, seed=0):
        g = torch.Generator(device=self.flat.device).manual_seed(seed)
        for n, v in self.views.items():
            if n.endswith(".kernel"):
                v.normal_(0.0, 1.0 / math.sqrt(math.prod(v.shape[:-1])), generator=g)
            elif n.endswith(".scale"):
                v.fill_(1.0)
            else:
                v.zero_()


def _add_conv(d, name, cin, cout, k):
    d[name + ".kernel"] = (k, k, cin, cout)
    d[name + ".bias"] = (cout,)


def _add_dense(d, name, cin, cout, bias=True):
    d[name + ".kernel"] = (cin, cout)
    if bias:
        d[name + ".bias"] = (cout,)


def _add_norm(d, name, c):
    d[name + ".scale"] = (c,)
    d[name + ".bias"] = (c,)


def add_resnet(d, name, cin, cout, temb_dim):
    _add_norm(d, name + ".norm1", cin)
    _add_conv(d, name + ".conv1", cin, cout, 3)
    if temb_dim:
        _add_dense(d, name + ".time_emb_proj", temb_dim, cout)
    _add_norm(d, name + ".norm2", cout)
    _add_conv(d, name + ".conv2", cout, cout, 3)
    if cin != cout:
        _add_conv(d, name + ".conv_shortcut", cin, cout, 1)


def _add_transformer(d, name, c, ctx, linear):
    _add_norm(d, name + ".norm", c)
    (_add_dense if linear else lambda dd, n, a, b: _add_conv(dd, n, a, b, 1))(d, name + ".proj_in", c, c)
    tb = name + ".transformer_blocks_0"
    for attn, kv in (("attn1", c), ("attn2", ctx)):
        _add_dense(d, f"{tb}.{attn}.to_q", c, c, bias=False)
        _add_dense(d, f"{tb}.{attn}.to_k", kv, c, bias=False)
        _add_dense(d, f"{tb}.{attn}.to_v", kv, c, bias=False)
        _add_dense(d, f"{tb}.{attn}.to_out_0", c, c)
    _add_dense(d, tb + ".ff.net_0.proj", c, 8 * c)
    _add_dense(d, tb + ".ff.net_2", 4 * c, c)
    for n in ("norm1", "norm2", "norm3"):
        _add_norm(d, f"{tb}.{n}", c)
    (_add_dense if linear else lambda dd, n, a, b: _add_conv(dd, n, a, b, 1))(d, name + ".proj_out", c, c)


def unet_param_shapes(cfg: UNetConfig):
    d = OrderedDict()
    boc = cfg.block_out_channels
    nlev = len(boc)
    temb = 4 * boc[0]
    _add_conv(d, "conv_in", cfg.in_channels, boc[0], 3)
    _add_dense(d, "time_embedding.linear_1", boc[0], temb)
    _add_dense(d, "time_embedding.linear_2", temb, temb)
    ch = boc[0]
    for i in range(nlev):
        for j in range(cfg.layers_per_block):
            add_resnet(d, f"down_blocks_{i}.resnets_{j}", ch, boc[i], temb)
            ch = boc[i]
            if cfg.cross_attn_down[i]:
                _add_transformer(d, f"down_blocks_{i}.attentions_{j}", ch, cfg.cross_attention_dim, cfg.use_linear_projection)
# ... 357 lines not shown
            if not inplace:
                return None
            c0, c1 = plan[len(plan) - 1 - len(cat_bufs)]
            buf = torch.empty(rows, c0 + c1, dtype=torch.float32, device=self.device)
            cat_bufs.append(buf)
            return buf[:, c0:]

        def up_dest(k):
            if not inplace or k >= len(plan):
                return None
            return cat_bufs[-1][:, :plan[k][0]]

        x = L.nchw_to_nhwc(sample[:Bh].contiguous())
        d0 = skip_dest(B * H * W)
        if d0 is not None:
            t, _, _ = L.conv2d(x, P["conv_in.kernel"], P["conv_in.bias"], Bh, H, W, Cin, boc[0], 3, out=d0[:Bh * H * W], ld_out=int(d0.stride(0)))
            if dup:
                n0 = Bh * H * W
                L.copy_cols(d0[:n0], d0[n0:], 0, n0, boc[0], ld_src=int(d0.stride(0)), ld_dst=int(d0.stride(0)))
            t_full = d0
        else:
            t, _, _ = L.conv2d(x, P["conv_in.kernel"], P["conv_in.bias"], Bh, H, W, Cin, boc[0], 3)
            t_full = twice(t)
        if tape is not None:
            tape.append(("head", dict(emb=emb, t1=t1, s1=s1, temb=temb, temb_act=temb_act, x=Act(x, B, H, W, Cin))))
        h_half = Act(t, Bh, H, W, boc[0])
        h = Act(t_full, B, H, W, boc[0])
        skips = [h]
        for i in range(nlev):
            for j in range(cfg.layers_per_block):
                if dup and i == 0 and j == 0:
                    r = resnet_forward(P, "down_blocks_0.resnets_0", h_half, temb_act if shared_t else temb_act[:Bh], G, 1e-5, None)
                    h = Act(twice(r.t), B, r.H, r.W, r.C)
                else:
                    emit = 0
                    if tape is None and i < nlev - 1 and j == cfg.layers_per_block - 1:
                        emit = L.planes_pay(P[f"down_blocks_{i}.downsamplers_0.conv.kernel"], boc[i], h.M)
                    h = resnet_forward(P, f"down_blocks_{i}.resnets_{j}", h, temb_act, G, 1e-5, tape,
                                       emit_planes=0 if cfg.cross_attn_down[i] else emit,
                                       dest=None if cfg.cross_attn_down[i] else skip_dest(h.M))
                if cfg.cross_attn_down[i]:
                    emit_t = 0
                    if tape is None and i < nlev - 1 and j == cfg.layers_per_block - 1:
                        emit_t = L.planes_pay(P[f"down_blocks_{i}.downsamplers_0.conv.kernel"], boc[i], h.M)
                    h = self._transformer(f"down_blocks_{i}.attentions_{j}", h, ctx, Lc, cfg.num_heads[i], tape, emit_planes=emit_t,
                                          dest=skip_dest(h.M))
                skips.append(h)
                if tape is not None:
                    tape.append(("skip_push", None))
            if i < nlev - 1:
                name = f"down_blocks_{i}.downsamplers_0.conv"
                src = h.pl if (h.pl is not None and L.planes_pay(P[name + ".kernel"], h.C, h.M) == h.pl.fmt + 1) else h.t
                skw = {} if (src is not h.t or h.ld is None) else dict(ld_src=h.ld)
                dd = skip_dest(B * (h.H // 2) * (h.W // 2))
                if dd is not None:
                    skw.update(out=dd, ld_out=int(dd.stride(0)))
                t, OH, OW = L.conv2d(src, P[name + ".kernel"], P[name + ".bias"], B, h.H, h.W, h.C, h.C, 3, stride=2, pad=1, **skw)
                if tape is not None:
                    tape.append(("down", dict(name=name, x=h)))
                    tape.append(("skip_push", None))
                h = Act(t, B, OH, OW, h.C)
                skips.append(h)
        h = resnet_forward(P, "mid_block.resnets_0", h, temb_act, G, 1e-5, tape)
        h = self._transformer("mid_block.attentions_0", h, ctx, Lc, cfg.num_heads[-1], tape)
        h = resnet_forward(P, "mid_block.resnets_1", h, temb_act, G, 1e-5, tape, dest=up_dest(0))
        kblk = 0
        for i in range(nlev):
            lvl = nlev - 1 - i
            for j in range(cfg.layers_per_block + 1):
                s = skips.pop()
                if inplace:
                    cat = cat_bufs.pop()
                    assert cat.shape == (B * h.HW, h.C + s.C) and h.t.data_ptr() == cat.data_ptr() and s.t.data_ptr() == cat.data_ptr() + 4 * h.C
                else:
                    cat = torch.empty(B * h.HW, h.C + s.C, dtype=torch.float32, device=self.device)
                    L.copy_cols(h.t, cat, 0, B * h.HW, h.C)
                    L.copy_cols(s.t, cat, h.C, B * h.HW, s.C)
                if tape is not None:
                    tape.append(("concat", dict(c0=h.C, c1=s.C)))
                kblk += 1
                emit = 0
                last_of_level = j == cfg.layers_per_block
                if tape is None and i < nlev - 1 and last_of_level:
                    emit = L.planes_pay(P[f"up_blocks_{i}.upsamplers_0.conv.kernel"], boc[lvl], B * h.HW)
                nxt = None if last_of_level else up_dest(kblk)
                h = resnet_forward(P, f"up_blocks_{i}.resnets_{j}", Act(cat, B, h.H, h.W, h.C + s.C), temb_act, G, 1e-5, tape,
                                   emit_planes=0 if cfg.cross_attn_down[lvl] else emit, dest=None if cfg.cross_attn_down[lvl] else nxt)
                if cfg.cross_attn_down[lvl]:
                    h = self._transformer(f"up_blocks_{i}.attentions_{j}", h, ctx, Lc, cfg.num_heads[lvl], tape, emit_planes=emit, dest=nxt)
            if i < nlev - 1:
                name = f"up_blocks_{i}.upsamplers_0.conv"
                src = h.pl if (h.pl is not None and L.planes_pay(P[name + ".kernel"], h.C, h.M) == h.pl.fmt + 1) else h.t
                dd = up_dest(kblk)
                t, OH, OW = L.conv2d(src, P[name + ".kernel"], P[name + ".bias"], B, h.H, h.W, h.C, h.C, 3, upsample=True,
                                     **({} if dd is None else dict(out=dd, ld_out=int(dd.stride(0)))))
                if tape is not None:
                    tape.append(("up", dict(name=name, x=h)))
                h = Act(t, B, OH, OW, h.C)
        hn, st = L.groupnorm(h.t, B, h.HW, P["conv_norm_out.scale"], P["conv_norm_out.bias"], G, 1e-5, True, return_stats=True,
                             planes=L.norm_planes(P["conv_out.kernel"], h.C, h.M, tape is not None) if tape is None else 0)
        t, _, _ = L.conv2d(hn, P["conv_out.kernel"], P["conv_out.bias"], B, h.H, h.W, h.C, cfg.out_channels, 3)
        if tape is not None:
            tape.append(("tail", dict(x=h, hn=hn, st=st)))
        return L.nhwc_to_nchw(t, B, cfg.out_channels, h.H, h.W)

    __call__ = forward

    def _concat_plan(self):
        cfg = self.cfg
        boc = cfg.block_out_channels
        nlev = len(boc)
        pushed = [boc[0]]
        for i in range(nlev):
            pushed += [boc[i]] * cfg.layers_per_block
            if i < nlev - 1:
                pushed.append(boc[i])
        plan, ch, rev = [], boc[-1], boc[::-1]
        for i in range(nlev):
            for _ in range(cfg.layers_per_block + 1):
                plan.append((ch, pushed.pop()))
                ch = rev[i]
        assert not pushed
        return plan

    def cross_attention_names(self):
        return [n[:-len(".to_k.kernel")] for n in self.params.views if n.endswith(".attn2.to_k.kernel")]

    def precompute_context(self, context):
        B, Lc, D = context.shape
        ctx = context.reshape(B * Lc, D).contiguous()
        for name in self.cross_attention_names():
            wk, wv = self.params[name + ".to_k.kernel"], self.params[name + ".to_v.kernel"]
            ent = self._ctx_kv.get((name, B * Lc))
            heads = self._heads_of(name)
            nb = 0
            if L.current_datapath() != "fp32" and (wk.shape[1] // heads) in (8, 16, 40, 64, 80) and os.environ.get("DDPO_CTX_IMAGES", "1") != "0":
                nb = int(L.load().ddpo_attention_kv_images_bytes(B, heads, Lc, wk.shape[1] // heads))
            if ent is None:
                kbuf = torch.empty(B * Lc, wk.shape[1], dtype=torch.float32, device=self.device)
                vbuf = torch.empty(B * Lc, wv.shape[1], dtype=torch.float32, device=self.device)
                ent = (kbuf, vbuf, torch.empty(nb, dtype=torch.uint8, device=self.device) if nb else None)
                self._ctx_kv[(name, B * Lc)] = ent
            elif ent[2] is None and nb:
                ent = (ent[0], ent[1], torch.empty(nb, dtype=torch.uint8, device=self.device))
                self._ctx_kv[(name, B * Lc)] = ent
            L.linear(ctx, wk, out=ent[0])
            L.linear(ctx, wv, out=ent[1])
            if ent[2] is not None:
                L.attention_kv_images(ent[0], ent[1], B, heads, Lc, wk.shape[1] // heads, out=ent[2])
        self._ctx_kv_active = True

    def release_context(self):
        self._ctx_kv_active = False
        self._graph_ctx_token = None

    def _heads_of(self, attn_name):
        cfg = self.cfg
        nlev = len(cfg.block_out_channels)
        if attn_name.startswith("down_blocks_"):
            return cfg.num_heads[int(attn_name.split("_")[2].split(".")[0])]
        if attn_name.startswith("up_blocks_"):
            return cfg.num_heads[nlev - 1 - int(attn_name.split("_")[2].split(".")[0])]
        return cfg.num_heads[-1]

    def time_proj_names(self):
        return [n[:-len(".time_emb_proj.kernel")] for n in self.params.views if n.endswith(".time_emb_proj.kernel")]

    def precompute_timesteps(self, timesteps):
        P = self.params
        ts = torch.as_tensor(timesteps, dtype=torch.int32, device=self.device).reshape(-1).contiguous()
        T = ts.numel()
        names = self.time_proj_names()
        widths = [P[n + ".time_emb_proj.bias"].numel() for n in names]
        total = sum(widths)
        ent = self._temb
        if ent is None or ent["table"].shape != (T, total):
            row = torch.zeros(1, total, dtype=torch.float32, device=self.device) if ent is None else ent["row"]
            views, off = {}, 0
# ... 168 lines not shown
```

### ddpo_amd/models/vae.py

```python
import math
from collections import OrderedDict
from dataclasses import dataclass
from typing import Tuple

import torch

from .. import lib as L
from .unet import Act, ParamStore, add_resnet, resnet_forward, _add_conv, _add_dense, _add_norm


@dataclass(frozen=True)
class VAEConfig:
    latent_channels: int = 4
    out_channels: int = 3
    block_out_channels: Tuple[int, ...] = (128, 256, 512, 512)
    layers_per_block: int = 2
    norm_groups: int = 32
    scaling_factor: float = 0.18215

    @staticmethod
    def named(name):
        if name in ("sd", "sd15", "sd21"):
            return VAEConfig()
        if name == "tiny":
# ... 3 lines not shown

def vae_decoder_param_shapes(cfg: VAEConfig):
    d = OrderedDict()
    boc = cfg.block_out_channels
    top = boc[-1]
    _add_conv(d, "post_quant_conv", cfg.latent_channels, cfg.latent_channels, 1)
    _add_conv(d, "decoder.conv_in", cfg.latent_channels, top, 3)
    add_resnet(d, "decoder.mid_block.resnets_0", top, top, 0)
    a = "decoder.mid_block.attentions_0"
    _add_norm(d, a + ".group_norm", top)
    for n in ("query", "key", "value", "proj_attn"):
        _add_dense(d, f"{a}.{n}", top, top)
    add_resnet(d, "decoder.mid_block.resnets_1", top, top, 0)
    ch = top
    for i, out_c in enumerate(boc[::-1]):
        for j in range(cfg.layers_per_block + 1):
            add_resnet(d, f"decoder.up_blocks_{i}.resnets_{j}", ch, out_c, 0)
            ch = out_c
        if i < len(boc) - 1:
            _add_conv(d, f"decoder.up_blocks_{i}.upsamplers_0.conv", ch, ch, 3)
    _add_norm(d, "decoder.conv_norm_out", boc[0])
    _add_conv(d, "decoder.conv_out", boc[0], cfg.out_channels, 3)
    return d


class VAEDecoder:
    def __init__(self, cfg: VAEConfig, device="cuda"):
        self.cfg = cfg
        self.device = torch.device(device)
        self.params = ParamStore(vae_decoder_param_shapes(cfg), self.device)
        self._out_pad = None

    def _padded_conv_out(self):
        if self._out_pad is None:
            k = self.params["decoder.conv_out.kernel"]
            b = self.params["decoder.conv_out.bias"]
            n4 = (self.cfg.out_channels + 3) // 4 * 4
            kp = torch.zeros(*k.shape[:3], n4, dtype=torch.float32, device=self.device)
            kp[..., : k.shape[3]] = k
            bp = torch.zeros(n4, dtype=torch.float32, device=self.device)
            bp[: b.numel()] = b
            self._out_pad = (kp, bp, n4)
        return self._out_pad

    def invalidate(self):
        self._out_pad = None

    def _mid_attention(self, x: Act):
        P = self.params
        a = "decoder.mid_block.attentions_0"
        B, N, C = x.B, x.HW, x.C
        t = L.groupnorm(x.t, B, N, P[a + ".group_norm.scale"], P[a + ".group_norm.bias"], self.cfg.norm_groups, 1e-6, False)
        q = L.linear(t, P[a + ".query.kernel"], P[a + ".query.bias"])
        k = L.linear(t, P[a + ".key.kernel"], P[a + ".key.bias"])
        v = L.linear(t, P[a + ".value.kernel"], P[a + ".value.bias"])
        o = torch.empty(B * N, C, dtype=torch.float32, device=self.device)
        scores = torch.empty(N, N, dtype=torch.float32, device=self.device)
        for b in range(B):
            sl = slice(b * N, (b + 1) * N)
            L.gemm_conv(q[sl], k[sl], M=N, N=N, K=C, w_trans=True, alpha=1.0 / math.sqrt(C), out=scores)
            L.softmax_rows_(scores)
            L.gemm_conv(scores, v[sl], M=N, N=C, K=N, out=o[sl])
        out = L.linear(o, P[a + ".proj_attn.kernel"], P[a + ".proj_attn.bias"], residual=x.t)
        return Act(out, B, x.H, x.W, C)

    def decode(self, latents):
        P, cfg = self.params, self.cfg
        B, Cl, H, W = latents.shape
        G = cfg.norm_groups
        z = L.nchw_to_nhwc(latents.contiguous())
        z, _, _ = L.conv2d(z, P["post_quant_conv.kernel"], P["post_quant_conv.bias"], B, H, W, Cl, Cl, 1,
                           alpha=1.0 / cfg.scaling_factor)
        top = cfg.block_out_channels[-1]
        t, _, _ = L.conv2d(z, P["decoder.conv_in.kernel"], P["decoder.conv_in.bias"], B, H, W, Cl, top, 3)
        h = Act(t, B, H, W, top)
        h = resnet_forward(P, "decoder.mid_block.resnets_0", h, None, G, 1e-6)
        h = self._mid_attention(h)
        h = resnet_forward(P, "decoder.mid_block.resnets_1", h, None, G, 1e-6)
        n = len(cfg.block_out_channels)
        for i in range(n):
            for j in range(cfg.layers_per_block + 1):
                h = resnet_forward(P, f"decoder.up_blocks_{i}.resnets_{j}", h, None, G, 1e-6)
            if i < n - 1:
                t, OH, OW = L.conv2d(h.t, P[f"decoder.up_blocks_{i}.upsamplers_0.conv.kernel"],
                                     P[f"decoder.up_blocks_{i}.upsamplers_0.conv.bias"], B, h.H, h.W, h.C, h.C, 3, upsample=True)
                h = Act(t, B, OH, OW, h.C)
        t = L.groupnorm(h.t, B, h.HW, P["decoder.conv_norm_out.scale"], P["decoder.conv_norm_out.bias"], G, 1e-6, True)
        kp, bp, n4 = self._padded_conv_out()
        t, _, _ = L.conv2d(t, kp, bp, B, h.H, h.W, h.C, n4, 3)
        img = t[:, : cfg.out_channels].contiguous()
        img = L.scale_shift_clip(img, 0.5, 0.5, 0.0, 1.0)
        return img.view(B, h.H, h.W, cfg.out_channels)


def vae_encoder_param_shapes(cfg: VAEConfig, in_channels=3):
    d = OrderedDict()
    boc = cfg.block_out_channels
    _add_conv(d, "encoder.conv_in", in_channels, boc[0], 3)
    ch = boc[0]
    for i, out_c in enumerate(boc):
        for j in range(cfg.layers_per_block):
            add_resnet(d, f"encoder.down_blocks_{i}.resnets_{j}", ch, out_c, 0)
            ch = out_c
        if i < len(boc) - 1:
            _add_conv(d, f"encoder.down_blocks_{i}.downsamplers_0.conv", ch, ch, 3)
    add_resnet(d, "encoder.mid_block.resnets_0", ch, ch, 0)
    a = "encoder.mid_block.attentions_0"
    _add_norm(d, a + ".group_norm", ch)
    for n in ("query", "key", "value", "proj_attn"):
        _add_dense(d, f"{a}.{n}", ch, ch)
    add_resnet(d, "encoder.mid_block.resnets_1", ch, ch, 0)
    _add_norm(d, "encoder.conv_norm_out", ch)
    _add_conv(d, "encoder.conv_out", ch, 2 * cfg.latent_channels, 3)
    _add_conv(d, "quant_conv", 2 * cfg.latent_channels, 2 * cfg.latent_channels, 1)
    return d


class VAEEncoder:

    def __init__(self, cfg: VAEConfig, device="cuda", in_channels=3):
        self.cfg = cfg
        self.device = torch.device(device)
        self.in_channels = in_channels
        self.params = ParamStore(vae_encoder_param_shapes(cfg, in_channels), self.device)
        self._in_pad = None

    def invalidate(self):
        self._in_pad = None

    def _padded_conv_in(self):
        if self._in_pad is None:
            k = self.params["encoder.conv_in.kernel"]
            c4 = (self.in_channels + 3) // 4 * 4
            kp = torch.zeros(k.shape[0], k.shape[1], c4, k.shape[3], dtype=torch.float32, device=self.device)
            kp[:, :, : k.shape[2]] = k
            self._in_pad = (kp, c4)
        return self._in_pad

    def encode(self, images):
        P, cfg = self.params, self.cfg
        B, H, W, Ci = images.shape
        G = cfg.norm_groups
        kp, c4 = self._padded_conv_in()
        x = torch.zeros(B * H * W, c4, dtype=torch.float32, device=self.device)
        x[:, :Ci] = (images.to(self.device, torch.float32).reshape(B * H * W, Ci) - 0.5) / 0.5
        boc = cfg.block_out_channels
        t, _, _ = L.conv2d(x, kp, P["encoder.conv_in.bias"], B, H, W, c4, boc[0], 3)
        h = Act(t, B, H, W, boc[0])
        n = len(boc)
        for i in range(n):
            for j in range(cfg.layers_per_block):
                h = resnet_forward(P, f"encoder.down_blocks_{i}.resnets_{j}", h, None, G, 1e-6)
            if i < n - 1:
                xp = torch.zeros(B, h.H + 1, h.W + 1, h.C, dtype=torch.float32, device=self.device)
                xp[:, : h.H, : h.W] = h.t.view(B, h.H, h.W, h.C)
                t, OH, OW = L.conv2d(xp.view(-1, h.C), P[f"encoder.down_blocks_{i}.downsamplers_0.conv.kernel"],
                                     P[f"encoder.down_blocks_{i}.downsamplers_0.conv.bias"], B, h.H + 1, h.W + 1, h.C, h.C, 3, stride=2, pad=0)
                h = Act(t, B, OH, OW, h.C)
        h = resnet_forward(P, "encoder.mid_block.resnets_0", h, None, G, 1e-6)
        h = self._mid_attention(h)
        h = resnet_forward(P, "encoder.mid_block.resnets_1", h, None, G, 1e-6)
        t = L.groupnorm(h.t, B, h.HW, P["encoder.conv_norm_out.scale"], P["encoder.conv_norm_out.bias"], G, 1e-6, True)
        c2 = 2 * cfg.latent_channels
        t, _, _ = L.conv2d(t, P["encoder.conv_out.kernel"], P["encoder.conv_out.bias"], B, h.H, h.W, h.C, c2, 3)
        m, _, _ = L.conv2d(t, P["quant_conv.kernel"], P["quant_conv.bias"], B, h.H, h.W, c2, c2, 1)
        m = m.view(B, h.H, h.W, c2)
        m[..., cfg.latent_channels:].clamp_(-30.0, 20.0)
        return m
# ... 19 lines not shown
```

### include/ddpo_hip.h

```cpp
#ifndef DDPO_HIP_H
#define DDPO_HIP_H
#include <stddef.h>
#include <stdint.h>
#ifdef __cplusplus
extern "C" {
#endif

#define DDPO_OK 0
#define DDPO_EINVAL (-1)
#define DDPO_ELAUNCH (-2)

#define DDPO_PRED_EPSILON 0
#define DDPO_PRED_V 1
#define DDPO_PRED_SAMPLE 2

int ddpo_abi_version(void);
size_t ddpo_sizeof_gemm_desc(void);
size_t ddpo_sizeof_ddim_consts(void);
int ddpo_gemm_tile_launch_counts(unsigned long long* out_host, int n);

int ddpo_threefry_bits_host(uint32_t k0, uint32_t k1, int64_t n, uint32_t* out_host);
int ddpo_threefry_normal(uint32_t k0, uint32_t k1, float* out, uint32_t* bits_out, int64_t n, void* stream);

typedef struct {
// ... 8 lines not shown
int ddpo_ddim_step_fwd(const float* eps_u, const float* eps_c, const float* x, const float* z,
                       const int32_t* ts, float guidance_scale, const ddpo_ddim_consts* c,
                       float* x_next, float* logp, int B, int chw, void* stream);

int ddpo_ddim_logprob_ppo_fwd_bwd(const float* eps_c, const float* eps_u, const float* x,
                                  const float* x_next, const int32_t* ts, const float* old_logp,
                                  const float* advantages, float guidance_scale, float clip_range,
                                  int train_cfg, const ddpo_ddim_consts* c, float* d_eps_c,
                                  float* d_eps_u, float* per_sample, float* info, int B, int chw,
                                  void* stream);
int ddpo_ddim_logprob_ppo_fwd_bwd_grouped(const float* eps_c, const float* eps_u, const float* x,
                                          const float* x_next, const int32_t* ts, const float* old_logp,
                                          const float* advantages, float guidance_scale, float clip_range,
                                          int train_cfg, const ddpo_ddim_consts* c, float* d_eps_c,
                                          float* d_eps_u, float* per_sample, float* info, int B, int group,
                                          int chw, void* stream);

int ddpo_rwr_noisy_latents(const float* moments, const float* e1, const float* noise, const int32_t* ts,
                           const float* alphas_cumprod, int num_train_timesteps, float scale, float* latents, float* noisy,
                           int B, int C, int hw, void* stream);
int ddpo_rwr_mse_fwd_bwd(const float* eps_c, const float* eps_u, const float* noise, const float* weights, float guidance_scale,
                         int train_cfg, float* d_eps_c, float* d_eps_u, float* per_sample, float* loss, int B, int chw,
                         void* stream);
int ddpo_grad_sqnorm(const float* g, int64_t n, double* out_sq, int zero_first, void* stream);
int ddpo_adamw_bf16mu_step(float* p, float* g, uint16_t* mu, float* nu, int64_t n,
                           const double* sqnorm_of_sum, double inv_n_acc, double lr, double b1, double b2,
                           double eps, double weight_decay, double max_grad_norm, int step_t,
                           int mu_decay_in_bf16, int zero_grad, void* stream);


size_t ddpo_groupnorm_ws_bytes(int B, int HW, int C, int G);
size_t ddpo_groupnorm_stats_floats(int B, int C, int G);
int ddpo_groupnorm_fwd(const float* x, int ldx, float* y, int ldy, const float* gamma, const float* beta,
                       int B, int HW, int C, int G, float eps, int fuse_silu, void* ws, float* stats, void* stream);
int ddpo_groupnorm_fwd_planes(const float* x, int ldx, uint16_t* y_hi, uint16_t* y_lo, int ldy, const float* gamma,
                              const float* beta, int B, int HW, int C, int G, float eps, int fuse_silu, void* ws,
                              float* stats, void* stream);
size_t ddpo_groupnorm_bwd_ws_bytes(int B, int HW, int C, int G);
int ddpo_groupnorm_bwd(const float* x, int ldx, const float* dy, int lddy, const float* stats, const float* gamma,
                       int B, int HW, int C, int G, int fuse_silu, const float* dx_add, int ld_add, float* dx, int lddx,
                       float* dgamma, float* dbeta, void* ws, void* stream);
int ddpo_layernorm_fwd(const float* x, float* y, const float* gamma, const float* beta, int rows, int C,
                       float eps, void* stream);
int ddpo_layernorm_fwd_planes(const float* x, uint16_t* y_hi, uint16_t* y_lo, const float* gamma, const float* beta,
                              int rows, int C, float eps, int kblocked, void* stream);
size_t ddpo_layernorm_bwd_ws_bytes(int rows, int C);
int ddpo_layernorm_bwd(const float* x, const float* dy, const float* gamma, int rows, int C, float eps,
                       const float* dx_add, float* dx, float* dgamma, float* dbeta, void* ws, void* stream);

typedef struct {
  const float* src; int ld_src;
  const float* w; int w_trans;
  const float* bias;
  const float* rowbias; int rows_per_batch; int ld_rowbias;
  const float* residual; int ld_res;
  float* out; int ld_out;
  float alpha;
  int M, N, K;
  int ksize, stride, pad, upsample;
  int B, H, W, Cin;
  int OH, OW;
  int w_dgrad;
  int ld_w;
  int splits;
  int accumulate;
  int epilogue;
  uint16_t* out_hi; uint16_t* out_lo; int ld_planes;
  int w_layout;
  const uint8_t* w_scale;
  int planes_fmt;
  float* colsum;
  float* aux_out;
} ddpo_gemm_desc;
int ddpo_gemm_conv_fwd(const ddpo_gemm_desc* d, void* stream);
int ddpo_gemm_conv_wgrad(const ddpo_gemm_desc* d, void* stream);

int ddpo_gemm_conv_fwd_bf16(const ddpo_gemm_desc* d, const uint16_t* w_hi, const uint16_t* w_lo, int ldw, int npass,
                            void* ws, size_t ws_bytes, void* stream);
int ddpo_gemm_conv_fwd_bf16_planes(const ddpo_gemm_desc* d, const uint16_t* a_hi, const uint16_t* a_lo, int lda,
                                   const uint16_t* w_hi, const uint16_t* w_lo, int ldw, void* ws, size_t ws_bytes,
                                   void* stream);
int ddpo_gemm_conv_fwd_f16mx_planes(const ddpo_gemm_desc* d, const uint16_t* a16, const uint16_t* a8, int lda,
                                    const uint16_t* w16, const uint16_t* w8, void* ws, size_t ws_bytes, void* stream);
int ddpo_pack_weights_f16mx(const float* w, int K, int N, uint16_t* w16, uint16_t* w8, uint8_t* scale, void* stream);
int ddpo_split_planes_f16mx(const float* x, int ldx, uint16_t* p16, uint16_t* p8, int ld_out, int64_t rows, int cols, void* stream);
int ddpo_pack_weights_bf16_kblocked(const float* w, int K, int N, uint16_t* fwd_hi, uint16_t* fwd_lo, void* stream);
int ddpo_pack_weights_bf16_kblocked_dgrad(const float* w, int taps, int Cin, int Cout, uint16_t* hi, uint16_t* lo, void* stream);
int ddpo_split_planes_bf16(const float* x, int ldx, uint16_t* hi, uint16_t* lo, int ld_out, int64_t rows, int cols,
                           void* stream);
int ddpo_gemm_conv_wgrad_bf16x3(const ddpo_gemm_desc* d, void* stream);
int ddpo_gemm_conv_wgrad_bf16x3_planes(const ddpo_gemm_desc* d, const uint16_t* a_hi, const uint16_t* a_lo,
                                       const uint16_t* dy_hi, const uint16_t* dy_lo, void* stream);
int ddpo_pack_weights_bf16(const float* w, int K, int N, int Kp, uint16_t* fwd_hi, uint16_t* fwd_lo,
                           uint16_t* bwd_hi, uint16_t* bwd_lo, void* stream);

int ddpo_attention_fwd(const float* q, int ldq, const float* k, int ldk, const float* v, int ldv,
                       float* o, int ldo, float* lse, int B, int heads, int Nq, int Nk, int d, float scale,
                       void* stream);
size_t ddpo_attention_fwd_bf16x3_ws_bytes(int B, int heads, int Nk, int d);
size_t ddpo_attention_kv_images_bytes(int B, int heads, int Nk, int d);
int ddpo_attention_pack_kv_bf16x3(const float* k, int ldk, const float* v, int ldv, void* images, size_t images_bytes,
                                  int B, int heads, int Nk, int d, void* stream);
int ddpo_attention_fwd_bf16x3_images(const float* q, int ldq, const void* images, size_t images_bytes, float* o, int ldo,
                                     float* lse, int B, int heads, int Nq, int Nk, int d, float scale, void* stream);
int ddpo_attention_fwd_bf16x3(const float* q, int ldq, const float* k, int ldk, const float* v, int ldv,
                              float* o, int ldo, float* lse, int B, int heads, int Nq, int Nk, int d, float scale,
                              void* ws, size_t ws_bytes, void* stream);
int ddpo_attention_bwd(const float* q, int ldq, const float* k, int ldk, const float* v, int ldv, const float* o,
                       const float* d_o, const float* lse, float* dvec, float* dq, float* dk, float* dv,
                       int B, int heads, int Nq, int Nk, int d, float scale, void* stream);

int ddpo_attention_bwd_bf16x3(const float* q, int ldq, const float* k, int ldk, const float* v, int ldv, const float* o,
                              const float* d_o, const float* lse, float* dvec, float* dq, float* dk, float* dv,
                              int B, int heads, int Nq, int Nk, int d, float scale, void* stream);

int ddpo_attention_fwd_f16p(const float* q, int ldq, const float* k, int ldk, const float* v, int ldv,
                            float* o, int ldo, float* lse, int B, int heads, int Nq, int Nk, int d, float scale,
                            void* ws, size_t ws_bytes, void* stream);
int ddpo_attention_pack_kv_f16p(const float* k, int ldk, const float* v, int ldv, void* images, size_t images_bytes, int B, int heads,
                                int Nk, int d, void* stream);
int ddpo_attention_fwd_f16p_images(const float* q, int ldq, const void* images, size_t images_bytes, float* o, int ldo,
                                   float* lse, int B, int heads, int Nq, int Nk, int d, float scale, void* stream);
int ddpo_attention_bwd_f16p(const float* q, int ldq, const float* k, int ldk, const float* v, int ldv, const float* o,
                            const float* d_o, const float* lse, float* dvec, float* dq, float* dk, float* dv,
                            int B, int heads, int Nq, int Nk, int d, float scale, void* stream);


int ddpo_attention_fwd_bf16x3_po(const float* q, int ldq, const float* k, int ldk, const float* v, int ldv, uint16_t* o_hi, uint16_t* o_lo,
                                 int ld_planes, float* lse, int B, int heads, int Nq, int Nk, int d, float scale, void* ws, size_t ws_bytes,
                                 void* stream);
int ddpo_attention_fwd_f16p_po(const float* q, int ldq, const float* k, int ldk, const float* v, int ldv, uint16_t* o_hi, uint16_t* o_lo,
                               int ld_planes, float* lse, int B, int heads, int Nq, int Nk, int d, float scale, void* ws, size_t ws_bytes,
                               void* stream);
int ddpo_attention_fwd_bf16x3_images_po(const float* q, int ldq, const void* images, size_t images_bytes, uint16_t* o_hi, uint16_t* o_lo,
                                        int ld_planes, float* lse, int B, int heads, int Nq, int Nk, int d, float scale, void* stream);
int ddpo_attention_fwd_f16p_images_po(const float* q, int ldq, const void* images, size_t images_bytes, uint16_t* o_hi, uint16_t* o_lo,
                                      int ld_planes, float* lse, int B, int heads, int Nq, int Nk, int d, float scale, void* stream);


int ddpo_geglu_fwd(const float* x, float* y, int64_t rows, int F, void* stream);
int ddpo_silu_fwd(const float* x, float* y, int64_t n, void* stream);
int ddpo_quick_gelu_fwd(const float* x, float* y, int64_t n, void* stream);
int ddpo_l2_normalize_rows(const float* x, float* y, int rows, int cols, void* stream);
int ddpo_attention_causal_fwd(const float* q, int ldq, const float* k, int ldk, const float* v, int ldv, float* o, int ldo,
                              int B, int heads, int N, int d, float scale, void* stream);
int ddpo_gather_rows(const float* table, int ld, int table_rows, const int32_t* idx, int rows, int cols, const float* add, int add_period,
                     float* out, void* stream);
int ddpo_cosine_rows(const float* a, const float* b, int rows, int cols, float scale, float* out, void* stream);
int ddpo_timestep_embedding(const int32_t* ts, float* out, int B, int dim, void* stream);
int ddpo_nchw_to_nhwc(const float* x, float* y, int B, int C, int HW, void* stream);
int ddpo_nhwc_to_nchw(const float* x, float* y, int B, int C, int HW, void* stream);
int ddpo_copy_cols(const float* src, int ld_src, float* dst, int ld_dst, int64_t rows, int cols, void* stream);
int ddpo_stage_cfg_inputs(const float* x, float* s_in, int64_t n, const float* row_src, float* row_dst, int row_n,
                          const int32_t* ts_src, int32_t* ts_dst, int ts_n, void* stream);
int ddpo_softmax_rows(float* x, int64_t rows, int cols, float scale, void* stream);
int ddpo_geglu_bwd(const float* x, const float* dy, float* dx, int64_t rows, int F, void* stream);
int ddpo_silu_bwd(const float* x, const float* dy, float* dx, int64_t n, void* stream);
int ddpo_colsum_accum(const float* x, int ldx, int64_t rows, int cols, int rows_per_seg, float* out, void* stream);
int ddpo_sumpool2x2(const float* x, float* y, int B, int H, int W, int C, void* stream);
int ddpo_add(const float* a, const float* b, float* out, int64_t n, void* stream);
int ddpo_scale_shift_clip(const float* x, float* y, int64_t n, float scale, float shift, float lo, float hi, void* stream);

typedef struct ddpo_lora_layer {
  const float* w0;
  float* w;
  const float* a;
// ... 15 lines not shown
```

Measured before the change: 4.198 images/sec.

## Fold nearest-upsample into 3x3 conv as four 2x2 phase convolutions

```diff
diff --git a/ddpo_amd/csrc/gemm_bf16.hip b/ddpo_amd/csrc/gemm_bf16.hip
--- a/ddpo_amd/csrc/gemm_bf16.hip
+++ b/ddpo_amd/csrc/gemm_bf16.hip
@@ -80,6 +80,10 @@
   *reinterpret_cast<uint2*>(d.out_lo + o) = l;
 }
 
+__device__ __forceinline__ int64_t fold_row(const ddpo_gemm_desc& d, int row, int ph) {
+  return 2 * (int64_t)row + 2 * (int64_t)d.W * (row / d.W) + (ph >> 1) * 2 * d.W + (ph & 1);
+}
+
 constexpr int epi_gcd(int a, int b) { return b == 0 ? a : epi_gcd(b, a % b); }
 template <int NIT, int LPR, int WTN, int NBMAX = 10>
 struct EpiRows {
@@ -137,7 +141,8 @@
       combine(d, cw, b0, row_base, col_base, lane);
     }
   }
-  __device__ __forceinline__ static void emit(const ddpo_gemm_desc& d, const float* cw, int row_base, int col_base, int lane) {
+  template <bool FOLD = false>
+  __device__ __forceinline__ static void emit(const ddpo_gemm_desc& d, const float* cw, int row_base, int col_base, int lane, int ph = 0) {
 #pragma unroll
     for (int b0 = 0; b0 < NIT; b0 += LB) {
       asm volatile("" : "+v"(lane));
@@ -152,6 +157,7 @@
         const int e = (b0 + i) * 64 + lane, rr = e / LPR;
         const int row = row_base + rr, col = col_base + (e - rr * LPR) * 4;
         if (row >= d.M || col >= d.N) continue;
+        if constexpr (FOLD) { st_out4(d.out + fold_row(d, row, ph) * d.ld_out + col, v[i]); continue; }
         if (d.out) st_out4(d.out + (int64_t)row * d.ld_out + col, v[i]);
         if (d.out_hi) store_planes4(d, row, col, v[i]);
       }
@@ -439,9 +445,9 @@
   return __builtin_amdgcn_make_buffer_rsrc(const_cast<void*>(p), 0, 0x7FFFFFFF, 0x00020000);
 }
 
-template <int BM, int BN, int NPASS, int ABL = 0, int WM = 2, int WN = 2, bool DEEP = true, int APL = 0>
-__global__ void __launch_bounds__(64 * WM * WN, (BM * BN <= 128 * 64 ? 3 : 1)) gemm_conv_bf16_buf_kernel(const ddpo_gemm_desc d, const uint16_t* __restrict__ w_hi,
-                                                                       const uint16_t* __restrict__ w_lo, int ldw, int tiles_m,
+template <int BM, int BN, int NPASS, int ABL = 0, int WM = 2, int WN = 2, bool DEEP = true, int APL = 0, bool FOLD = false>
+__global__ void __launch_bounds__(64 * WM * WN, (BM * BN <= 128 * 64 ? 3 : 1)) gemm_conv_bf16_buf_kernel(const ddpo_gemm_desc d, const uint16_t* __restrict__ w_hi_,
+                                                                       const uint16_t* __restrict__ w_lo_, int ldw, int tiles_m,
                                                                        int tiles_n, int nblk, int kt_per_split,
                                                                        float* __restrict__ part) {
   constexpr int BK = BF_BK;
@@ -455,6 +461,10 @@
   static_assert(BM % AR == 0 && WTM % 32 == 0 && WTN % 32 == 0, "tile / wave-grid mismatch");
   constexpr bool MX = NPASS == 4;
   static_assert(!MX || APL == 3 || APL == 7, "the f16mx datapath exists on the plane-fed 128-row tiles (APL 3) and on the tall tile (APL 7)");
+  static_assert(!FOLD || (APL != 0 && APL != 6), "folded up-sampler phases exist on the plane-fed kernels");
+  const int ph = FOLD ? (int)blockIdx.z : 0;
+  const uint16_t* __restrict__ w_hi = FOLD ? w_hi_ + (int64_t)ph * d.K * d.N : w_hi_;
+  const uint16_t* __restrict__ w_lo = (FOLD && w_lo_) ? w_lo_ + (int64_t)ph * d.K * d.N : w_lo_;
   constexpr int NPL = (NPASS == 3 || NPASS == 4) ? 2 : 1;
   constexpr int A_BYTES = BM * 64, B_BYTES = BN * 64;
   extern __shared__ __attribute__((aligned(16))) char smem[];
@@ -479,8 +489,8 @@
   const int m0 = tile_m * BM, n0 = tile_n * BN;
 
   const bool conv = d.ksize > 0;
-  const int VH = d.upsample ? d.H * 2 : d.H, VW = d.upsample ? d.W * 2 : d.W;
-  const bool zins = d.upsample == 2;
+  const int VH = (!FOLD && d.upsample) ? d.H * 2 : d.H, VW = (!FOLD && d.upsample) ? d.W * 2 : d.W;
+  const bool zins = !FOLD && d.upsample == 2;
   const int cin = conv ? d.Cin : d.K;
   const int ntaps = conv ? d.ksize * d.ksize : 1;
 
@@ -532,7 +542,7 @@
 #pragma unroll
     for (int j = 0; j < TN; ++j) {
       const int n = n0 + wn * WTN + j * 32 + (lane & 31);
-      const int sc = n < d.N ? (int)d.w_scale[n] : 127;
+      const int sc = n < d.N ? (int)d.w_scale[(FOLD ? ph * d.N : 0) + n] : 127;
       mx_sbp[j >> 2] |= (khalf ? sc : sc - 11) << (8 * (j & 3));
     }
   }
@@ -589,8 +599,8 @@
         const int mm = valid ? m : 0;
         const int b = mm / ohw, rem = mm - b * ohw;
         const int oy = rem / d.OW, ox = rem - oy * d.OW;
-        aiy0[i] = valid ? oy * d.stride - d.pad : -(1 << 24);
-        aix0[i] = ox * d.stride - d.pad;
+        aiy0[i] = valid ? (FOLD ? oy - 1 + (ph >> 1) : oy * d.stride - d.pad) : -(1 << 24);
+        aix0[i] = FOLD ? ox - 1 + (ph & 1) : ox * d.stride - d.pad;
         apix[i] = b * d.H * d.W;
         avoff[i] = BUF_OOB;
       } else {
@@ -599,13 +609,13 @@
       }
     }
     auto set_tap = [&](int tap) {
-      const int ky = d.ksize == 3 ? (tap * 11) >> 5 : 0;
-      const int kx = d.ksize == 3 ? tap - ky * 3 : 0;
+      const int ky = FOLD ? tap >> 1 : (d.ksize == 3 ? (tap * 11) >> 5 : 0);
+      const int kx = FOLD ? tap & 1 : (d.ksize == 3 ? tap - ky * 3 : 0);
 #pragma unroll
       for (int i = 0; i < NA; ++i) {
         const int iy = aiy0[i] + ky, ix = aix0[i] + kx;
         const bool ok = (unsigned)iy < (unsigned)VH && (unsigned)ix < (unsigned)VW && !(zins && ((iy | ix) & 1));
-        const int sy = d.upsample ? (iy >> 1) : iy, sx = d.upsample ? (ix >> 1) : ix;
+        const int sy = (!FOLD && d.upsample) ? (iy >> 1) : iy, sx = (!FOLD && d.upsample) ? (ix >> 1) : ix;
         const uint32_t off = (uint32_t)(apix[i] + sy * d.W + sx) * a_row_b + lc16;
         avoff[i] = ok ? off : BUF_OOB;
       }
@@ -1074,7 +1084,7 @@
       static_assert((32 * LPR) % 64 == 0, "32-row pass must be a whole number of wave instructions");
       __syncthreads();
       float* cw = reinterpret_cast<float*>(smem) + wid * (32 * WTN);
-      float* pp = part ? part + (int64_t)blockIdx.y * d.M * d.N : nullptr;
+      float* pp = part ? part + ((int64_t)ph * gridDim.y + blockIdx.y) * d.M * d.N : nullptr;
       using Epi = EpiRows<NIT, LPR, WTN, 5>;
       Epi ep;
       const int colb = n0 + wn * WTN;
@@ -1136,7 +1146,7 @@
         } else {
           if (ih == 0) { ep.init(d, colb, lane); ep.fetch(d, 0, rowb, colb, lane); }
           ep.combine_all(d, cw, rowb, colb, lane);
-          Epi::emit(d, cw, rowb, colb, lane);
+          Epi::template emit<FOLD>(d, cw, rowb, colb, lane, ph);
         }
       };
       pass(std::integral_constant<int, 0>{});
@@ -1190,16 +1200,16 @@
       return;
     }
     if (part) {
-      Epi::partials(d, cw, part + (int64_t)blockIdx.y * d.M * d.N, rowb, colb, lane);
+      Epi::partials(d, cw, part + ((int64_t)ph * gridDim.y + blockIdx.y) * d.M * d.N, rowb, colb, lane);
     } else {
       ep.combine_all(d, cw, rowb, colb, lane);
-      Epi::emit(d, cw, rowb, colb, lane);
+      Epi::template emit<FOLD>(d, cw, rowb, colb, lane, ph);
     }
     DBG_T(3);
     return;
   }
   if (part) {
-    float* pp = part + (int64_t)blockIdx.y * d.M * d.N;
+    float* pp = part + ((int64_t)ph * gridDim.y + blockIdx.y) * d.M * d.N;
 #pragma unroll
     for (int i = 0; i < TM; ++i)
 #pragma unroll
@@ -1230,7 +1240,7 @@
         float v = d.alpha * acc[i][j][r] + bv;
         if (d.rowbias) v += d.rowbias[(int64_t)(row / d.rows_per_batch) * d.ld_rowbias + col];
         if (d.residual) v += d.residual[(int64_t)row * d.ld_res + col];
-        d.out[(int64_t)row * d.ld_out + col] = v;
+        d.out[(FOLD ? fold_row(d, row, ph) : (int64_t)row) * d.ld_out + col] = v;
       }
     }
   }
@@ -1240,6 +1250,9 @@
 __global__ void __launch_bounds__(256) splitk_reduce_kernel(const ddpo_gemm_desc d, const float* __restrict__ part, int splits) {
   const int n4 = d.N >> 2;
   const int64_t total = (int64_t)d.M * n4, mn = (int64_t)d.M * d.N;
+  const bool fold = d.upsample == 3;
+  const int ph = blockIdx.y;
+  part += (int64_t)ph * splits * mn;
   for (int64_t i = (int64_t)blockIdx.x * blockDim.x + threadIdx.x; i < total; i += (int64_t)gridDim.x * blockDim.x) {
     const int row = (int)(i / n4), col = (int)(i - (int64_t)row * n4) << 2;
     float4 a = *reinterpret_cast<const float4*>(part + (int64_t)row * d.N + col);
@@ -1254,7 +1267,7 @@
       if (d.rowbias) x += d.rowbias[(int64_t)(row / d.rows_per_batch) * d.ld_rowbias + col + e];
       if (d.residual) x += d.residual[(int64_t)row * d.ld_res + col + e];
       v[e] = x;
-      if (d.out) d.out[(int64_t)row * d.ld_out + col + e] = x;
+      if (d.out) d.out[(fold ? fold_row(d, row, ph) : (int64_t)row) * d.ld_out + col + e] = x;
     }
     if (d.out_hi) store_planes4(d, row, col, make_float4(v[0], v[1], v[2], v[3]));
   }
@@ -1304,18 +1317,20 @@
 extern "C" void ddpo_debug_force_generic_gemm(int on) { g_force_generic = on != 0; }
 #endif
 
-template <int BM, int BN, int NPASS, int WM = 2, int WN = 2, int APL = 0>
+template <int BM, int BN, int NPASS, int WM = 2, int WN = 2, int APL = 0, bool FOLD = false>
 static int launch_bf16(const ddpo_gemm_desc& d, const uint16_t* w_hi, const uint16_t* w_lo, int ldw, float* ws, size_t ws_bytes,
                        hipStream_t st) {
+  constexpr int NPH = FOLD ? 4 : 1;
   const int tiles_m = (d.M + BM - 1) / BM, tiles_n = (d.N + BN - 1) / BN;
   const int nblk = tiles_m * tiles_n;
+  const int ngrid = nblk * NPH;
   const int nk_total = (d.K + BF_BK - 1) / BF_BK;
   int splits = 1;
-  if (ws && nblk < 192 && nk_total >= 32 && (d.N & 3) == 0 && d.epilogue == 0) {
-    splits = (384 + nblk - 1) / nblk;
+  if (ws && ngrid < 192 && nk_total >= 32 && (d.N & 3) == 0 && d.epilogue == 0) {
+    splits = (384 + ngrid - 1) / ngrid;
     if (splits > 8) splits = 8;
     if (splits > nk_total / 8) splits = nk_total / 8;
-    while (splits > 1 && (size_t)splits * d.M * d.N * sizeof(float) > ws_bytes) --splits;
+    while (splits > 1 && (size_t)NPH * splits * d.M * d.N * sizeof(float) > ws_bytes) --splits;
   }
   int ktps = (nk_total + splits - 1) / splits;
   ktps = (ktps + 1) & ~1;
@@ -1332,14 +1347,14 @@
       (void)hipFuncSetAttribute(reinterpret_cast<const void*>(&gemm_conv_bf16_kernel<BM, BN, NPASS, false>),
                                 hipFuncAttributeMaxDynamicSharedMemorySize, (int)lds);
     }
-    (void)hipFuncSetAttribute(reinterpret_cast<const void*>(&gemm_conv_bf16_buf_kernel<BM, BN, NPASS, 0, WM, WN, true, APL>),
+    (void)hipFuncSetAttribute(reinterpret_cast<const void*>(&gemm_conv_bf16_buf_kernel<BM, BN, NPASS, 0, WM, WN, true, APL, FOLD>),
                               hipFuncAttributeMaxDynamicSharedMemorySize, (int)lds);
     attr_set = true;
   }
   count_tile(BN == 128 ? TC_128 : TC_64);
   if constexpr (NPASS == 4) count_tile(TC_MX);
   if constexpr (APL != 0) {
-    hipLaunchKernelGGL((gemm_conv_bf16_buf_kernel<BM, BN, NPASS, 0, WM, WN, true, APL>), dim3(nblk, splits), dim3(64 * WM * WN), lds, st, d, w_hi,
+    hipLaunchKernelGGL((gemm_conv_bf16_buf_kernel<BM, BN, NPASS, 0, WM, WN, true, APL, FOLD>), dim3(nblk, splits, NPH), dim3(64 * WM * WN), lds, st, d, w_hi,
                        w_lo, ldw, tiles_m, tiles_n, nblk, ktps, part);
   } else {
     if (!buf_path_ok(d, ldw)) count_tile(TC_GENERIC);
@@ -1358,15 +1373,15 @@
     int64_t blocks = ((int64_t)d.M * (d.N >> 2) + 255) / 256;
     if (blocks > 4096) blocks = 4096;
     count_tile(TC_SPLITK_REDUCE);
-    hipLaunchKernelGGL(splitk_reduce_kernel, dim3((int)blocks), dim3(256), 0, st, d, part, splits);
+    hipLaunchKernelGGL(splitk_reduce_kernel, dim3((int)blocks, NPH), dim3(256), 0, st, d, part, splits);
     DDPO_LAUNCH_CHECK();
   }
   return DDPO_OK;
 }
 
 
-static int wide_splits(const ddpo_gemm_desc& d, bool have_ws, size_t ws_bytes) {
-  const int nblk = ((d.M + 127) / 128) * ((d.N + 319) / 320);
+static int wide_splits(const ddpo_gemm_desc& d, bool have_ws, size_t ws_bytes, int nph = 1) {
+  const int nblk = nph * ((d.M + 127) / 128) * ((d.N + 319) / 320);
   const int nk_total = d.K / BF_BK;
   int splits = 1;
   if (have_ws && nblk <= 192 && nk_total >= 16) {
@@ -1374,19 +1389,20 @@
     if (splits > 8) splits = 8;
     if (splits > nk_total / 8) splits = nk_total / 8;
     if (splits < 1) splits = 1;
-    while (splits > 1 && (size_t)splits * d.M * d.N * sizeof(float) > ws_bytes) --splits;
+    while (splits > 1 && (size_t)nph * splits * d.M * d.N * sizeof(float) > ws_bytes) --splits;
   }
   return splits;
 }
 
-template <int NPASS, int APL = 0>
+template <int NPASS, int APL = 0, bool FOLD = false>
 static int launch_bf16_wide(const ddpo_gemm_desc& d, const uint16_t* w_hi, const uint16_t* w_lo, int ldw, float* ws, size_t ws_bytes,
                             hipStream_t st) {
   constexpr int BM = 128, BN = 320, WM = 4, WN = 2;
+  constexpr int NPH = FOLD ? 4 : 1;
   const int tiles_m = (d.M + BM - 1) / BM, tiles_n = (d.N + BN - 1) / BN;
   const int nblk = tiles_m * tiles_n;
   const int nk_total = d.K / BF_BK;
-  int splits = wide_splits(d, ws != nullptr, ws_bytes);
+  int splits = wide_splits(d, ws != nullptr, ws_bytes, NPH);
   int ktps = (nk_total + splits - 1) / splits;
   ktps = (ktps + 1) & ~1;
   splits = (nk_total + ktps - 1) / ktps;
@@ -1394,26 +1410,26 @@
   const size_t lds = (size_t)BM * BN * 4;
   static bool attr_set = false;
   if (!attr_set) {
-    (void)hipFuncSetAttribute(reinterpret_cast<const void*>(&gemm_conv_bf16_buf_kernel<BM, BN, NPASS, 0, WM, WN, true, APL>),
+    (void)hipFuncSetAttribute(reinterpret_cast<const void*>(&gemm_conv_bf16_buf_kernel<BM, BN, NPASS, 0, WM, WN, true, APL, FOLD>),
                               hipFuncAttributeMaxDynamicSharedMemorySize, (int)lds);
     attr_set = true;
   }
   count_tile(TC_WIDE);
   if constexpr (NPASS == 4) count_tile(TC_MX);
-  hipLaunchKernelGGL((gemm_conv_bf16_buf_kernel<BM, BN, NPASS, 0, WM, WN, true, APL>), dim3(nblk, splits), dim3(64 * WM * WN), lds, st, d, w_hi,
+  hipLaunchKernelGGL((gemm_conv_bf16_buf_kernel<BM, BN, NPASS, 0, WM, WN, true, APL, FOLD>), dim3(nblk, splits, NPH), dim3(64 * WM * WN), lds, st, d, w_hi,
                      w_lo, ldw, tiles_m, tiles_n, nblk, ktps, part);
   DDPO_LAUNCH_CHECK();
   if (splits > 1) {
     int64_t blocks = ((int64_t)d.M * (d.N >> 2) + 255) / 256;
     if (blocks > 4096) blocks = 4096;
     count_tile(TC_SPLITK_REDUCE);
-    hipLaunchKernelGGL(splitk_reduce_kernel, dim3((int)blocks), dim3(256), 0, st, d, part, splits);
+    hipLaunchKernelGGL(splitk_reduce_kernel, dim3((int)blocks, NPH), dim3(256), 0, st, d, part, splits);
     DDPO_LAUNCH_CHECK();
   }
   return DDPO_OK;
 }
 
-template <int APL, int NPASS = 3>
+template <int APL, int NPASS = 3, bool FOLD = false>
 static int launch_bf16_tall(const ddpo_gemm_desc& d, const uint16_t* w_hi, const uint16_t* w_lo, int ldw, hipStream_t st) {
   constexpr int BM = 256, BN = 320, WM = 4, WN = 2;
   const int tiles_m = (d.M + BM - 1) / BM, tiles_n = (d.N + BN - 1) / BN;
@@ -1422,17 +1438,18 @@
   const size_t lds = 8 * 32 * 160 * 4;
   static bool attr_set = false;
   if (!attr_set) {
-    (void)hipFuncSetAttribute(reinterpret_cast<const void*>(&gemm_conv_bf16_buf_kernel<BM, BN, NPASS, 0, WM, WN, true, APL>),
+    (void)hipFuncSetAttribute(reinterpret_cast<const void*>(&gemm_conv_bf16_buf_kernel<BM, BN, NPASS, 0, WM, WN, true, APL, FOLD>),
                               hipFuncAttributeMaxDynamicSharedMemorySize, (int)lds);
     attr_set = true;
   }
   count_tile(TC_TALL);
-  hipLaunchKernelGGL((gemm_conv_bf16_buf_kernel<BM, BN, NPASS, 0, WM, WN, true, APL>), dim3(nblk, 1), dim3(64 * WM * WN), lds, st, d, w_hi, w_lo, ldw,
+  hipLaunchKernelGGL((gemm_conv_bf16_buf_kernel<BM, BN, NPASS, 0, WM, WN, true, APL, FOLD>), dim3(nblk, 1, FOLD ? 4 : 1), dim3(64 * WM * WN), lds, st, d, w_hi, w_lo, ldw,
                      tiles_m, tiles_n, nblk, nk_total, (float*)nullptr);
   DDPO_LAUNCH_CHECK();
   return DDPO_OK;
 }
 
+template <bool FOLD = false>
 static int launch_mx_tall(const ddpo_gemm_desc& d, const uint16_t* w16, const uint16_t* w8, hipStream_t st) {
   constexpr int BM = 256, BN = 320, WM = 4, WN = 2;
   const int tiles_m = (d.M + BM - 1) / BM, tiles_n = (d.N + BN - 1) / BN;
@@ -1441,22 +1458,25 @@
   const size_t lds = 8 * 32 * 160 * 4;
   static bool attr_set = false;
   if (!attr_set) {
-    (void)hipFuncSetAttribute(reinterpret_cast<const void*>(&gemm_conv_bf16_buf_kernel<BM, BN, 4, 0, WM, WN, true, 7>),
+    (void)hipFuncSetAttribute(reinterpret_cast<const void*>(&gemm_conv_bf16_buf_kernel<BM, BN, 4, 0, WM, WN, true, 7, FOLD>),
                               hipFuncAttributeMaxDynamicSharedMemorySize, (int)lds);
     attr_set = true;
   }
   count_tile(TC_TALL);
   count_tile(TC_MX);
-  hipLaunchKernelGGL((gemm_conv_bf16_buf_kernel<BM, BN, 4, 0, WM, WN, true, 7>), dim3(nblk, 1), dim3(64 * WM * WN), lds, st, d, w16, w8, 0,
+  hipLaunchKernelGGL((gemm_conv_bf16_buf_kernel<BM, BN, 4, 0, WM, WN, true, 7, FOLD>), dim3(nblk, 1, FOLD ? 4 : 1), dim3(64 * WM * WN), lds, st, d, w16, w8, 0,
                      tiles_m, tiles_n, nblk, nk_total, (float*)nullptr);
   DDPO_LAUNCH_CHECK();
   return DDPO_OK;
 }
 
-template <int APL>
+template <int APL, bool FOLD = false>
 static int dispatch_bf16(const ddpo_gemm_desc& d, const uint16_t* w_hi, const uint16_t* w_lo, int ldw, int npass, void* ws, size_t ws_bytes,
                          hipStream_t st) {
-  if (d.epilogue != 0) {
+  static_assert(!FOLD || APL == 3, "folded up-sampler phases exist on the plane-fed kernels");
+  constexpr int NPH = FOLD ? 4 : 1;
+  if constexpr (FOLD) { if (d.epilogue != 0 || (npass != 1 && npass != 3 && npass != 4)) return DDPO_EINVAL; }
+  if constexpr (!FOLD) if (d.epilogue != 0) {
     if ((d.epilogue != 1 && d.epilogue != 2) || (d.N & 127) || !buf_path_ok(d, ldw) || d.rowbias || d.residual || d.alpha != 1.0f || d.w_dgrad) return DDPO_EINVAL;
     if ((d.ld_out & 3) || (reinterpret_cast<uintptr_t>(d.out) & 15) || (d.bias && (reinterpret_cast<uintptr_t>(d.bias) & 15))) return DDPO_EINVAL;
     if (reinterpret_cast<uintptr_t>(d.aux_out) & 15) return DDPO_EINVAL;
@@ -1478,47 +1498,54 @@
   constexpr int wide_mode = 1;
   if constexpr (APL != 0) {
     constexpr int tall_mode = 1;
-    const long ntall = (long)((d.M + 255) / 256) * (d.N / 320), nwide = (long)((d.M + 127) / 128) * (d.N / 320);
+    const long ntall = (long)NPH * ((d.M + 255) / 256) * (d.N / 320), nwide = (long)NPH * ((d.M + 127) / 128) * (d.N / 320);
     const double eff_tall = (double)ntall / (double)(((ntall + 255) / 256) * 256), eff_wide = (double)nwide / (double)(((nwide + 255) / 256) * 256);
     if (tall_mode && npass == 3 && d.N % 320 == 0 && d.epilogue == 0 && ntall >= 200 && eff_tall * 1.08 >= eff_wide)
-      return launch_bf16_tall<5>(d, w_hi, w_lo, ldw, st);
+      return launch_bf16_tall<5, 3, FOLD>(d, w_hi, w_lo, ldw, st);
     if constexpr (APL == 3) {
       if (npass == 1 && d.N % 320 == 0 && d.epilogue == 0 && ntall >= 200 && eff_tall * 1.08 >= eff_wide)
-        return launch_bf16_tall<8, 1>(d, w_hi, w_lo, ldw, st);
-      if (npass == 5 && d.N % 320 == 0 && d.epilogue == 0 && ntall >= 200 && eff_tall * 1.08 >= eff_wide)
-        return launch_bf16_tall<8, 5>(d, w_hi, w_lo, ldw, st);
+        return launch_bf16_tall<8, 1, FOLD>(d, w_hi, w_lo, ldw, st);
+      if constexpr (!FOLD)
+        if (npass == 5 && d.N % 320 == 0 && d.epilogue == 0 && ntall >= 200 && eff_tall * 1.08 >= eff_wide)
+          return launch_bf16_tall<8, 5>(d, w_hi, w_lo, ldw, st);
       const char* mx_tall_env = getenv("DDPO_MX_TALL");
       if (npass == 4 && !(mx_tall_env && mx_tall_env[0] == '0') && d.N % 320 == 0 && d.epilogue == 0 && ntall >= 200 && eff_tall * 1.08 >= eff_wide)
-        return launch_mx_tall(d, w_hi, w_lo, st);
-    }
-  }
-  const int wsplits = wide_splits(d, wsf != nullptr, ws_bytes);
-  if (wide_mode && d.N % 320 == 0 && d.M >= 512 && buf_path_ok(d, ldw) && !(d.K / BF_BK < 16 && d.N > 1280) &&
-      (long)((d.M + 127) / 128) * (d.N / 320) * wsplits >= 200 &&
+        return launch_mx_tall<FOLD>(d, w_hi, w_lo, st);
+    }
+  }
+  const int wsplits = wide_splits(d, wsf != nullptr, ws_bytes, NPH);
+  if (wide_mode && d.N % 320 == 0 && (long)NPH * d.M >= 512 && buf_path_ok(d, ldw) && !(d.K / BF_BK < 16 && d.N > 1280) &&
+      (long)NPH * ((d.M + 127) / 128) * (d.N / 320) * wsplits >= 200 &&
       !(wsplits > 1 && d.K / BF_BK < 64)) {
     if constexpr (APL == 3) {
-      if (npass == 4) return launch_bf16_wide<4, 3>(d, w_hi, w_lo, ldw, wsf, ws_bytes, st);
-      if (npass == 1) return launch_bf16_wide<1, 3>(d, w_hi, w_lo, ldw, wsf, ws_bytes, st);
-      if (npass == 5) return launch_bf16_wide<5, 3>(d, w_hi, w_lo, ldw, wsf, ws_bytes, st);
-    }
-    return npass == 3 ? launch_bf16_wide<3, APL>(d, w_hi, w_lo, ldw, wsf, ws_bytes, st) : launch_bf16_wide<1>(d, w_hi, w_lo, ldw, wsf, ws_bytes, st);
-  }
-  const long t128 = (long)((d.M + 127) / 128) * ((d.N + 127) / 128);
+      if (npass == 4) return launch_bf16_wide<4, 3, FOLD>(d, w_hi, w_lo, ldw, wsf, ws_bytes, st);
+      if (npass == 1) return launch_bf16_wide<1, 3, FOLD>(d, w_hi, w_lo, ldw, wsf, ws_bytes, st);
+      if constexpr (!FOLD) if (npass == 5) return launch_bf16_wide<5, 3>(d, w_hi, w_lo, ldw, wsf, ws_bytes, st);
+    }
+    if constexpr (FOLD) return launch_bf16_wide<3, APL, true>(d, w_hi, w_lo, ldw, wsf, ws_bytes, st);
+    else return npass == 3 ? launch_bf16_wide<3, APL>(d, w_hi, w_lo, ldw, wsf, ws_bytes, st) : launch_bf16_wide<1>(d, w_hi, w_lo, ldw, wsf, ws_bytes, st);
+  }
+  const long t128 = (long)NPH * ((d.M + 127) / 128) * ((d.N + 127) / 128);
   constexpr long big_min = 256;
   constexpr int mid64 = 1;
   const bool mid_short = mid64 && t128 < 512 && d.K / BF_BK <= 64;
   const bool big = (d.N % 128 == 0) && t128 >= big_min && !mid_short;
   if constexpr (APL == 3) {
     if (npass == 4)
-      return big ? launch_bf16<128, 128, 4, 2, 2, 3>(d, w_hi, w_lo, ldw, wsf, ws_bytes, st) : launch_bf16<128, 64, 4, 2, 2, 3>(d, w_hi, w_lo, ldw, wsf, ws_bytes, st);
+      return big ? launch_bf16<128, 128, 4, 2, 2, 3, FOLD>(d, w_hi, w_lo, ldw, wsf, ws_bytes, st) : launch_bf16<128, 64, 4, 2, 2, 3, FOLD>(d, w_hi, w_lo, ldw, wsf, ws_bytes, st);
     if (npass == 1)
-      return big ? launch_bf16<128, 128, 1, 2, 2, 3>(d, w_hi, w_lo, ldw, wsf, ws_bytes, st) : launch_bf16<128, 64, 1, 2, 2, 3>(d, w_hi, w_lo, ldw, wsf, ws_bytes, st);
-    if (npass == 5)
-      return big ? launch_bf16<128, 128, 5, 2, 2, 3>(d, w_hi, w_lo, ldw, wsf, ws_bytes, st) : launch_bf16<128, 64, 5, 2, 2, 3>(d, w_hi, w_lo, ldw, wsf, ws_bytes, st);
-  }
-  if (npass == 3)
-    return big ? launch_bf16<128, 128, 3, 2, 2, APL>(d, w_hi, w_lo, ldw, wsf, ws_bytes, st) : launch_bf16<128, 64, 3, 2, 2, APL>(d, w_hi, w_lo, ldw, wsf, ws_bytes, st);
-  return big ? launch_bf16<128, 128, 1>(d, w_hi, w_lo, ldw, wsf, ws_bytes, st) : launch_bf16<128, 64, 1>(d, w_hi, w_lo, ldw, wsf, ws_bytes, st);
+      return big ? launch_bf16<128, 128, 1, 2, 2, 3, FOLD>(d, w_hi, w_lo, ldw, wsf, ws_bytes, st) : launch_bf16<128, 64, 1, 2, 2, 3, FOLD>(d, w_hi, w_lo, ldw, wsf, ws_bytes, st);
+    if constexpr (!FOLD)
+      if (npass == 5)
+        return big ? launch_bf16<128, 128, 5, 2, 2, 3>(d, w_hi, w_lo, ldw, wsf, ws_bytes, st) : launch_bf16<128, 64, 5, 2, 2, 3>(d, w_hi, w_lo, ldw, wsf, ws_bytes, st);
+  }
+  if constexpr (FOLD) {
+    return big ? launch_bf16<128, 128, 3, 2, 2, APL, true>(d, w_hi, w_lo, ldw, wsf, ws_bytes, st) : launch_bf16<128, 64, 3, 2, 2, APL, true>(d, w_hi, w_lo, ldw, wsf, ws_bytes, st);
+  } else {
+    if (npass == 3)
+      return big ? launch_bf16<128, 128, 3, 2, 2, APL>(d, w_hi, w_lo, ldw, wsf, ws_bytes, st) : launch_bf16<128, 64, 3, 2, 2, APL>(d, w_hi, w_lo, ldw, wsf, ws_bytes, st);
+    return big ? launch_bf16<128, 128, 1>(d, w_hi, w_lo, ldw, wsf, ws_bytes, st) : launch_bf16<128, 64, 1>(d, w_hi, w_lo, ldw, wsf, ws_bytes, st);
+  }
 }
 
 extern "C" int ddpo_gemm_conv_fwd_bf16(const ddpo_gemm_desc* dp, const uint16_t* w_hi, const uint16_t* w_lo, int ldw, int npass,
@@ -1599,6 +1626,69 @@
   { const char* e = getenv("DDPO_DBG_ABL"); if (e) d.splits |= atoi(e) << 4; }
 #endif
   return dispatch_bf16<3>(d, w16, w8, 0, npass, ws, ws_bytes, as_stream(stream));
+}
+
+extern "C" int ddpo_conv_up2x_folded_fwd(const ddpo_gemm_desc* dp, const uint16_t* a_hi, const uint16_t* a_lo, int lda, const uint16_t* w_hi,
+                                         const uint16_t* w_lo, int f16mx, void* ws, size_t ws_bytes, void* stream) {
+  if (!dp || !a_hi || !w_hi || (a_lo == nullptr) != (w_lo == nullptr)) return DDPO_EINVAL;
+  if (f16mx && (!a_lo || !dp->w_scale)) return DDPO_EINVAL;
+  const int npass = f16mx ? 4 : (a_lo ? 3 : 1);
+  ddpo_gemm_desc d = *dp;
+  if (d.B <= 0 || d.H <= 0 || d.W <= 0 || d.Cin <= 0 || d.N <= 0 || (d.Cin % BF_BK) || (d.N & 3)) return DDPO_EINVAL;
+  if ((int64_t)d.B * d.H * d.W * 4 > 0x7FFFFFFF || (int64_t)d.Cin * 4 > 0x7FFFFFFF) return DDPO_EINVAL;
+  if (lda < 0 || (lda & (f16mx ? 31 : 7)) || (lda && lda < d.Cin)) return DDPO_EINVAL;
+  if (!d.out || d.out_hi || d.out_lo || d.rowbias || d.residual || d.epilogue || d.w_dgrad || d.aux_out) return DDPO_EINVAL;
+  if (d.ld_out < d.N || (d.ld_out & 3) || (reinterpret_cast<uintptr_t>(d.out) & 15) || (d.bias && (reinterpret_cast<uintptr_t>(d.bias) & 15))) return DDPO_EINVAL;
+  if ((reinterpret_cast<uintptr_t>(a_hi) | reinterpret_cast<uintptr_t>(a_lo) | reinterpret_cast<uintptr_t>(w_hi) | reinterpret_cast<uintptr_t>(w_lo)) & 15)
+    return DDPO_EINVAL;
+  d.M = d.B * d.H * d.W; d.K = 4 * d.Cin;
+  d.alpha = 1.0f;
+  d.OH = d.H; d.OW = d.W;
+  d.ksize = 2; d.stride = 1; d.pad = 1; d.upsample = 3;
+  d.w_layout = 1; d.planes_fmt = 0; d.ld_planes = 0;
+  d.src = reinterpret_cast<const float*>(a_hi);
+  d.w = reinterpret_cast<const float*>(a_lo);
+  d.ld_src = lda;
+  if (!f16mx) d.w_scale = nullptr;
+  if (!buf_path_ok(d, 0) || (int64_t)4 * d.K * d.N * 2 >= 0x7FFFFFFF) return DDPO_EINVAL;
+  d.splits = 1;
+  return dispatch_bf16<3, true>(d, w_hi, w_lo, 0, npass, ws, ws_bytes, as_stream(stream));
+}
+
+__global__ void __launch_bounds__(256) fold_up2x_weights_kernel(const float* __restrict__ w, int64_t cn, float* __restrict__ wf) {
+  const int64_t i = (int64_t)blockIdx.x * 256 + threadIdx.x;
+  if (i >= cn) return;
+  float v[3][3];
+#pragma unroll
+  for (int ky = 0; ky < 3; ++ky)
+#pragma unroll
+    for (int kx = 0; kx < 3; ++kx) v[ky][kx] = w[(ky * 3 + kx) * cn + i];
+#pragma unroll
+  for (int ph = 0; ph < 4; ++ph)
+#pragma unroll
+    for (int t = 0; t < 4; ++t) {
+      const int py = ph >> 1, px = ph & 1, ty = t >> 1, tx = t & 1;
+      const int y0 = py ? (ty ? 2 : 0) : (ty ? 1 : 0), y1 = py ? (ty ? 2 : 1) : (ty ? 2 : 0);
+      const int x0 = px ? (tx ? 2 : 0) : (tx ? 1 : 0), x1 = px ? (tx ? 2 : 1) : (tx ? 2 : 0);
+      float sum = 0.f;
+      bool first = true;
+#pragma unroll
+      for (int ky = 0; ky < 3; ++ky)
+#pragma unroll
+        for (int kx = 0; kx < 3; ++kx) {
+          if (ky < y0 || ky > y1 || kx < x0 || kx > x1) continue;
+          sum = first ? v[ky][kx] : sum + v[ky][kx];
+          first = false;
+        }
+      wf[(ph * 4 + t) * cn + i] = sum;
+    }
+}
+extern "C" int ddpo_fold_up2x_weights(const float* w, int Cin, int Cout, float* wf, void* stream) {
+  if (!w || !wf || Cin <= 0 || Cout <= 0) return DDPO_EINVAL;
+  const int64_t cn = (int64_t)Cin * Cout;
+  hipLaunchKernelGGL(fold_up2x_weights_kernel, dim3((unsigned)((cn + 255) / 256)), dim3(256), 0, as_stream(stream), w, cn, wf);
+  DDPO_LAUNCH_CHECK();
+  return DDPO_OK;
 }
 
 __global__ void __launch_bounds__(256) pack_weights_kernel(const float* __restrict__ w, int K, int N, int Kp,
diff --git a/ddpo_amd/lib.py b/ddpo_amd/lib.py
--- a/ddpo_amd/lib.py
+++ b/ddpo_amd/lib.py
@@ -82,6 +82,8 @@
     "ddpo_pack_weights_f16mx": (c_int, [c_void_p, c_int, c_int, c_void_p, c_void_p, c_void_p, c_void_p]),
     "ddpo_split_planes_f16mx": (c_int, [c_void_p, c_int, c_void_p, c_void_p, c_int, c_int64, c_int, c_void_p]),
     "ddpo_gemm_conv_fwd_f16mx_planes": (c_int, [POINTER(GemmDesc), c_void_p, c_void_p, c_int, c_void_p, c_void_p, c_void_p, c_size_t, c_void_p]),
+    "ddpo_fold_up2x_weights": (c_int, [c_void_p, c_int, c_int, c_void_p, c_void_p]),
+    "ddpo_conv_up2x_folded_fwd": (c_int, [POINTER(GemmDesc), c_void_p, c_void_p, c_int, c_void_p, c_void_p, c_int, c_void_p, c_size_t, c_void_p]),
     "ddpo_attention_fwd": (c_int, [c_void_p, c_int, c_void_p, c_int, c_void_p, c_int, c_void_p, c_int, c_void_p, c_int, c_int,
                                    c_int, c_int, c_int, c_float, c_void_p]),
     "ddpo_attention_kv_images_bytes": (c_size_t, [c_int, c_int, c_int, c_int]),
@@ -619,6 +621,8 @@
         ent["bwd"] = (mk(K, N), mk(K, N))
     if "geglu" in ent:
         ent["geglu"]["stale"] = True
+    if "fold" in ent:
+        ent["fold"]["stale"] = True
     fh, fl, _ = ent["fwd"]
     bh, bl = ent["bwd"] if ent["bwd"] is not None else (None, None)
     if _mx() and K % 32 == 0 and K >= MX_MIN_K:
@@ -636,6 +640,139 @@
     else:
         _check(load().ddpo_pack_weights_bf16(_p(w), K, N, Kp, _p(fh), _p(fl), _p(bh), _p(bl), _stream()), "ddpo_pack_weights_bf16")
     return ent
+
+
+UP2X_FOLD = os.environ.get("DDPO_UP2X_FOLD", "1") == "1"
+
+
+def fold_up2x_kernel_reference(w):
+    groups = (((0,), (1, 2)), ((0, 1), (2,)))
+    out = w.new_zeros((4, 2, 2) + tuple(w.shape[2:]))
+    for py in range(2):
+        for px in range(2):
+            for ty in range(2):
+                for tx in range(2):
+                    acc = None
+                    for ky in groups[py][ty]:
+                        for kx in groups[px][tx]:
+                            acc = w[ky, kx].clone() if acc is None else acc + w[ky, kx]
+                    out[py * 2 + px, ty, tx] = acc
+    return out
+
+
+def conv_up2x_folded_reference(x, w):
+    B, H, W, _ = x.shape
+    wf = fold_up2x_kernel_reference(w)
+    xp = torch.nn.functional.pad(x, (0, 0, 1, 1, 1, 1))
+    out = x.new_zeros(B, 2 * H, 2 * W, w.shape[3])
+    for py in range(2):
+        for px in range(2):
+            acc = 0
+            for ty in range(2):
+                for tx in range(2):
+                    oy, ox = ty - 1 + py, tx - 1 + px
+                    acc = acc + xp[:, 1 + oy:1 + oy + H, 1 + ox:1 + ox + W] @ wf[py * 2 + px, ty, tx]
+            out[:, py::2, px::2] = acc
+    return out
+
+
+def pack_weights_up2x_folded(w):
+    ent = PACKED.get(w.data_ptr())
+    if ent is None:
+        raise DdpoHipError("pack_weights_up2x_folded: pack_weights(w) first")
+    C, N = int(w.shape[2]), int(w.shape[3])
+    if not (UP2X_FOLD and w.dim() == 4 and w.shape[0] == 3 and w.shape[1] == 3 and C % 32 == 0 and N % 4 == 0 and W_KBLOCKED):
+        ent.pop("fold", None)
+        return None
+    K, Kb = 4 * C, 4 * C // 32
+    fo = ent.get("fold")
+    if fo is None or fo["K"] != K or fo["N"] != N:
+        mk = lambda: torch.zeros(4, Kb, N, 32, dtype=torch.int16, device=w.device)
+        fo = ent["fold"] = dict(K=K, N=N, hi=mk(), lo=mk())
+    wf = torch.empty(4, K, N, dtype=torch.float32, device=w.device)
+    _check(load().ddpo_fold_up2x_weights(_p(w), C, N, _p(wf), _stream()), "ddpo_fold_up2x_weights")
+    mx = _mx() and K >= MX_MIN_K
+    if mx and "mx" not in fo:
+        fo["mx"] = dict(w16=torch.zeros(4, Kb, N, 32, dtype=torch.int16, device=w.device), w8=torch.zeros(4, Kb, N, 64, dtype=torch.uint8, device=w.device),
+                        scale=torch.zeros(4, N, dtype=torch.uint8, device=w.device))
+    if not mx:
+        fo.pop("mx", None)
+    for ph in range(4):
+        _check(load().ddpo_pack_weights_bf16_kblocked(_p(wf[ph]), K, N, _p(fo["hi"][ph]), _p(fo["lo"][ph]), _stream()), "ddpo_pack_weights_bf16_kblocked")
+        if mx:
+            m = fo["mx"]
+            _check(load().ddpo_pack_weights_f16mx(_p(wf[ph]), K, N, _p(m["w16"][ph]), _p(m["w8"][ph]), _p(m["scale"][ph]), _stream()), "ddpo_pack_weights_f16mx")
+    fo["stale"] = False
+    return fo
+
+
+def up2x_fold_ok(w, cin, rows):
+    if not UP2X_FOLD or current_datapath() == "fp32" or cin % 32 or (_mx() and not MX_CROSS):
+        return False
+    ent = PACKED.get(w.data_ptr())
+    if ent is None or "fold" not in ent:
+        return False
+    fo = ent["fold"]
+    if fo.get("stale", True):
+        return False
+    if _mx() and fo["K"] >= MX_MIN_K and "mx" not in fo:
+        return False
+    lim = 0x7FFFFFFF
+    return rows * cin * 4 < lim and 4 * fo["N"] * fo["K"] * 2 < lim and rows * 4 < lim
+
+
+def up2x_planes_pay(w, cin, rows):
+    if not up2x_fold_ok(w, cin, rows):
+        return planes_pay(w, cin, rows)
+    if not (PLANES and _planes_dp()):
+        return 0
+    return 2 if (_mx() and "mx" in PACKED[w.data_ptr()]["fold"]) else 1
+
+
+def conv2d_up2x_folded(x, w, bias, B, H, W, Cin, Cout, out=None, ld_out=None):
+    rows = B * H * W
+    if not up2x_fold_ok(w, Cin, rows):
+        raise DdpoHipError("conv2d_up2x_folded: no folded planes for this layer / datapath (check up2x_fold_ok)")
+    fo = PACKED[w.data_ptr()]["fold"]
+    if fo["K"] != 4 * Cin or fo["N"] != Cout:
+        raise DdpoHipError("conv2d_up2x_folded: geometry does not match the registered kernel")
+    mxl = _mx() and "mx" in fo
+    if isinstance(x, Planes):
+        pl = x
+        if pl.fmt != int(mxl) or pl.rows != rows or pl.C != Cin:
+            raise DdpoHipError("activation planes of the wrong format / shape for this layer (ask up2x_planes_pay)")
+    else:
+        if not (x.dim() == 2 and x.shape[0] == rows and x.shape[1] == Cin and x.stride(1) == 1):
+            raise DdpoHipError("conv2d_up2x_folded needs its fp32 input as a (rows, channels) tensor or row-strided view")
+        pl = split_planes(x, fmt=1 if mxl else 0)
+    M = 4 * rows
+    if out is None:
+        out = torch.empty(M, Cout, dtype=torch.float32, device=pl.device)
+    d = GemmDesc()
+    d.bias = bias.data_ptr() if bias is not None else None
+    d.out = out.data_ptr(); d.ld_out = int(ld_out if ld_out is not None else Cout)
+    d.alpha = 1.0
+    d.N = int(Cout)
+    d.B, d.H, d.W, d.Cin = int(B), int(H), int(W), int(Cin)
+    if PROFILE is not None:
+        e0, e1 = torch.cuda.Event(enable_timing=True), torch.cuda.Event(enable_timing=True)
+        e0.record()
+    ws = _scratch(SPLITK_WS_BYTES, pl.device, "splitk")
+    one = not _x3()
+    if mxl:
+        m = fo["mx"]
+        d.w_scale = m["scale"].data_ptr()
+        wh, wl = m["w16"], m["w8"]
+    else:
+        wh, wl = fo["hi"], (None if one else fo["lo"])
+    _check(load().ddpo_conv_up2x_folded_fwd(byref(d), _p(pl.hi), None if (one and not mxl) else _p(pl.lo), pl.ld, _p(wh), None if wl is None else _p(wl),
+                                            int(mxl), _p(ws), SPLITK_WS_BYTES, _stream()), "ddpo_conv_up2x_folded_fwd")
+    if PROFILE is not None:
+        e1.record()
+        K = 4 * Cin
+        io_bytes = 4.0 * rows * Cin + (4.0 if _x3() else 2.0) * 4 * K * Cout + 4.0 * M * Cout
+        PROFILE.append((e0, e1, 2.0 * M * Cout * K, "f16mx" if mxl else ("bf16x3" if _x3() else current_datapath()), io_bytes))
+    return out, 2 * H, 2 * W
 
 
 def _pack_dgrad_planes(w, ent):
diff --git a/ddpo_amd/models/unet.py b/ddpo_amd/models/unet.py
--- a/ddpo_amd/models/unet.py
+++ b/ddpo_amd/models/unet.py
@@ -78,6 +78,8 @@
                 if n not in sel or not n.endswith(".kernel"):
                     continue
                 L.pack_weights(v, bwd=bwd)
+                if n.endswith(".upsamplers_0.conv.kernel"):
+                    L.pack_weights_up2x_folded(v)
                 if n.endswith(".ff.net_0.proj.kernel"):
                     L.pack_weights_geglu(v, self.views[n[:-len("kernel")] + "bias"])
                 m = re.search(r"\.attn1\.to_[qkv]\.kernel$", n)
@@ -89,6 +91,8 @@
         for n, v in self.views.items():
             if n.endswith(".kernel"):
                 L.pack_weights(v, bwd=bwd)
+                if n.endswith(".upsamplers_0.conv.kernel"):
+                    L.pack_weights_up2x_folded(v)
                 if n.endswith(".ff.net_0.proj.kernel"):
                     L.pack_weights_geglu(v, self.views[n[:-len("kernel")] + "bias"])
                 if QKV_FUSED and n.endswith(".attn1.to_q.kernel"):
@@ -612,7 +616,7 @@
                 emit = 0
                 last_of_level = j == cfg.layers_per_block
                 if tape is None and i < nlev - 1 and last_of_level:
-                    emit = L.planes_pay(P[f"up_blocks_{i}.upsamplers_0.conv.kernel"], boc[lvl], B * h.HW)
+                    emit = L.up2x_planes_pay(P[f"up_blocks_{i}.upsamplers_0.conv.kernel"], boc[lvl], B * h.HW)
                 nxt = None if last_of_level else up_dest(kblk)
                 h = resnet_forward(P, f"up_blocks_{i}.resnets_{j}", Act(cat, B, h.H, h.W, h.C + s.C), temb_act, G, 1e-5, tape,
                                    emit_planes=0 if cfg.cross_attn_down[lvl] else emit, dest=None if cfg.cross_attn_down[lvl] else nxt)
@@ -620,10 +624,13 @@
                     h = self._transformer(f"up_blocks_{i}.attentions_{j}", h, ctx, Lc, cfg.num_heads[lvl], tape, emit_planes=emit, dest=nxt)
             if i < nlev - 1:
                 name = f"up_blocks_{i}.upsamplers_0.conv"
-                src = h.pl if (h.pl is not None and L.planes_pay(P[name + ".kernel"], h.C, h.M) == h.pl.fmt + 1) else h.t
+                src = h.pl if (h.pl is not None and L.up2x_planes_pay(P[name + ".kernel"], h.C, h.M) == h.pl.fmt + 1) else h.t
                 dd = up_dest(kblk)
-                t, OH, OW = L.conv2d(src, P[name + ".kernel"], P[name + ".bias"], B, h.H, h.W, h.C, h.C, 3, upsample=True,
-                                     **({} if dd is None else dict(out=dd, ld_out=int(dd.stride(0)))))
+                dkw = {} if dd is None else dict(out=dd, ld_out=int(dd.stride(0)))
+                if L.up2x_fold_ok(P[name + ".kernel"], h.C, h.M):
+                    t, OH, OW = L.conv2d_up2x_folded(src, P[name + ".kernel"], P[name + ".bias"], B, h.H, h.W, h.C, h.C, **dkw)
+                else:
+                    t, OH, OW = L.conv2d(src, P[name + ".kernel"], P[name + ".bias"], B, h.H, h.W, h.C, h.C, 3, upsample=True, **dkw)
                 if tape is not None:
                     tape.append(("up", dict(name=name, x=h)))
                 h = Act(t, B, OH, OW, h.C)
diff --git a/ddpo_amd/models/vae.py b/ddpo_amd/models/vae.py
--- a/ddpo_amd/models/vae.py
+++ b/ddpo_amd/models/vae.py
@@ -109,8 +109,11 @@
             for j in range(cfg.layers_per_block + 1):
                 h = resnet_forward(P, f"decoder.up_blocks_{i}.resnets_{j}", h, None, G, 1e-6)
             if i < n - 1:
-                t, OH, OW = L.conv2d(h.t, P[f"decoder.up_blocks_{i}.upsamplers_0.conv.kernel"],
-                                     P[f"decoder.up_blocks_{i}.upsamplers_0.conv.bias"], B, h.H, h.W, h.C, h.C, 3, upsample=True)
+                uk, ub = P[f"decoder.up_blocks_{i}.upsamplers_0.conv.kernel"], P[f"decoder.up_blocks_{i}.upsamplers_0.conv.bias"]
+                if L.up2x_fold_ok(uk, h.C, h.M):
+                    t, OH, OW = L.conv2d_up2x_folded(h.t, uk, ub, B, h.H, h.W, h.C, h.C)
+                else:
+                    t, OH, OW = L.conv2d(h.t, uk, ub, B, h.H, h.W, h.C, h.C, 3, upsample=True)
                 h = Act(t, B, OH, OW, h.C)
         t = L.groupnorm(h.t, B, h.HW, P["decoder.conv_norm_out.scale"], P["decoder.conv_norm_out.bias"], G, 1e-6, True)
         kp, bp, n4 = self._padded_conv_out()
diff --git a/include/ddpo_hip.h b/include/ddpo_hip.h
--- a/include/ddpo_hip.h
+++ b/include/ddpo_hip.h
@@ -114,6 +114,9 @@
                                    void* stream);
 int ddpo_gemm_conv_fwd_f16mx_planes(const ddpo_gemm_desc* d, const uint16_t* a16, const uint16_t* a8, int lda,
                                     const uint16_t* w16, const uint16_t* w8, void* ws, size_t ws_bytes, void* stream);
+int ddpo_fold_up2x_weights(const float* w, int Cin, int Cout, float* wf, void* stream);
+int ddpo_conv_up2x_folded_fwd(const ddpo_gemm_desc* d, const uint16_t* a_hi, const uint16_t* a_lo, int lda, const uint16_t* w_hi,
+                              const uint16_t* w_lo, int f16mx, void* ws, size_t ws_bytes, void* stream);
 int ddpo_pack_weights_f16mx(const float* w, int K, int N, uint16_t* w16, uint16_t* w8, uint8_t* scale, void* stream);
 int ddpo_split_planes_f16mx(const float* x, int ldx, uint16_t* p16, uint16_t* p8, int ld_out, int64_t rows, int cols, void* stream);
 int ddpo_pack_weights_bf16_kblocked(const float* w, int K, int N, uint16_t* fwd_hi, uint16_t* fwd_lo, void* stream);
```

Result: faster. 4.308 images/sec, median of 6 (+2.6%).
